# AbrahamSanders/realtime-codec-agent

Hardware: NVIDIA B200
Metric: encode audio-sec/sec (higher is better)
Workload: dtype bf16

## Files before the change

### realtime-codec-agent_b200/csrc/elementwise.cuh

```cuda
#pragma once
#include "gemm_sm100.cuh"

namespace mc {

template <int KT>
__global__ void __launch_bounds__(256)
conv_first_kernel(const float* __restrict__ wav, long long ld, int T, int B, int T0, int s0, int C0,
                  const float* __restrict__ w , const float* __restrict__ bias,
                  __nv_bfloat16* __restrict__ out, int pad_rows) {
  pdl_launch_dependents();
  pdl_wait();
  const int cgroups = C0 / 8;
  const int cg = threadIdx.x % cgroups;
  const int slot = threadIdx.x / cgroups;
  const int frames_per_block = blockDim.x / cgroups;
  float wr[KT][8], br[8];
#pragma unroll
  for (int j = 0; j < KT; ++j) {
    const float4 a = __ldg(reinterpret_cast<const float4*>(w + j * C0 + cg * 8));
    const float4 c = __ldg(reinterpret_cast<const float4*>(w + j * C0 + cg * 8 + 4));
    wr[j][0] = a.x; wr[j][1] = a.y; wr[j][2] = a.z; wr[j][3] = a.w;
    wr[j][4] = c.x; wr[j][5] = c.y; wr[j][6] = c.z; wr[j][7] = c.w;
  }
#pragma unroll
  for (int c = 0; c < 8; ++c) br[c] = __ldg(bias + cg * 8 + c);
  const long long total = static_cast<long long>(B) * T0;
  for (long long bt = blockIdx.x * static_cast<long long>(frames_per_block) + slot; bt < total;
       bt += static_cast<long long>(gridDim.x) * frames_per_block) {
    const int t = static_cast<int>(bt % T0);
    const int b = static_cast<int>(bt / T0);
    const float* x = wav + b * ld;
    float acc[8];
#pragma unroll
    for (int c = 0; c < 8; ++c) acc[c] = br[c];
#pragma unroll
    for (int j = 0; j < KT; ++j) {
      const int n = t * s0 + j - s0;
      const float xv = (n >= 0 && n < T) ? __ldg(x + n) : 0.0f;
#pragma unroll
      for (int c = 0; c < 8; ++c) acc[c] = fmaf(xv, wr[j][c], acc[c]);
    }
    uint4 o;
    o.x = pack_bf16x2(gelu_tanh_f(acc[0]), gelu_tanh_f(acc[1]));
    o.y = pack_bf16x2(gelu_tanh_f(acc[2]), gelu_tanh_f(acc[3]));
    o.z = pack_bf16x2(gelu_tanh_f(acc[4]), gelu_tanh_f(acc[5]));
    o.w = pack_bf16x2(gelu_tanh_f(acc[6]), gelu_tanh_f(acc[7]));
    __nv_bfloat16* dst = out + ((static_cast<long long>(b) * (pad_rows + T0) + pad_rows + t) * C0 + cg * 8);
    *reinterpret_cast<uint4*>(dst) = o;
  }
}

__global__ void rmsnorm_kernel(const float* __restrict__ x, const float* __restrict__ gamma,
                               __nv_bfloat16* __restrict__ out, int M, int d, float eps, int grp_in,
                               long long grp_stride, long long grp_off) {
  pdl_launch_dependents();
  pdl_wait();
  const int warps_per_block = blockDim.x >> 5;
  const int lane = threadIdx.x & 31;
  for (int row = blockIdx.x * warps_per_block + (threadIdx.x >> 5); row < M; row += gridDim.x * warps_per_block) {
    const float4* xr = reinterpret_cast<const float4*>(x + static_cast<long long>(row) * d);
    const int n4 = d >> 2;
    float ss = 0.0f;
    for (int i = lane; i < n4; i += 32) {
      const float4 v = xr[i];
      ss += v.x * v.x + v.y * v.y + v.z * v.z + v.w * v.w;
    }
#pragma unroll
    for (int o = 16; o > 0; o >>= 1) ss += __shfl_xor_sync(0xffffffffu, ss, o);
    const float inv = rsqrtf(ss / static_cast<float>(d) + eps);
    const int grp = row / grp_in;
    const long long obase = static_cast<long long>(grp) * grp_stride + grp_off + static_cast<long long>(row - grp * grp_in) * d;
    uint2* orow_p = reinterpret_cast<uint2*>(out + obase);
    const float4* g4 = reinterpret_cast<const float4*>(gamma);
    for (int i = lane; i < n4; i += 32) {
      const float4 v = xr[i];
      const float4 g = __ldg(g4 + i);
      uint2 o;
      o.x = pack_bf16x2(v.x * inv * g.x, v.y * inv * g.y);
      o.y = pack_bf16x2(v.z * inv * g.z, v.w * inv * g.w);
      orow_p[i] = o;
    }
  }
}

template <int NV>
__global__ void __launch_bounds__(256)
rmsnorm_rows_kernel(const float* __restrict__ x, const float* __restrict__ gamma, __nv_bfloat16* __restrict__ out, int M,
                    float eps, int grp_in, long long grp_stride, long long grp_off) {
  pdl_launch_dependents();
  pdl_wait();
  constexpr int d = NV * 128;
  const int warps_per_block = blockDim.x >> 5;
  const int lane = threadIdx.x & 31;
  float4 g[NV];
#pragma unroll
  for (int u = 0; u < NV; ++u) g[u] = __ldg(reinterpret_cast<const float4*>(gamma) + lane + 32 * u);
  for (int row = blockIdx.x * warps_per_block + (threadIdx.x >> 5); row < M; row += gridDim.x * warps_per_block) {
    const float4* xr = reinterpret_cast<const float4*>(x + static_cast<long long>(row) * d);
    float4 v[NV];
#pragma unroll
    for (int u = 0; u < NV; ++u) v[u] = xr[lane + 32 * u];
    float ss = 0.0f;
#pragma unroll
    for (int u = 0; u < NV; ++u) ss += v[u].x * v[u].x + v[u].y * v[u].y + v[u].z * v[u].z + v[u].w * v[u].w;
#pragma unroll
    for (int o = 16; o > 0; o >>= 1) ss += __shfl_xor_sync(0xffffffffu, ss, o);
    const float inv = rsqrtf(ss / static_cast<float>(d) + eps);
    const int grp = row / grp_in;
    const long long obase = static_cast<long long>(grp) * grp_stride + grp_off + static_cast<long long>(row - grp * grp_in) * d;
    uint2* orow_p = reinterpret_cast<uint2*>(out + obase);
#pragma unroll
    for (int u = 0; u < NV; ++u) {
      uint2 o;
      o.x = pack_bf16x2(v[u].x * inv * g[u].x, v[u].y * inv * g[u].y);
      o.y = pack_bf16x2(v[u].z * inv * g[u].z, v[u].w * inv * g[u].w);
      orow_p[lane + 32 * u] = o;
    }
  }
}

__global__ void compact_rows_kernel(const float4* __restrict__ x, float4* __restrict__ y, int B, int r_in, int r_out,
                                    int d4) {
  pdl_launch_dependents();
  pdl_wait();
  const long long total = static_cast<long long>(B) * r_out * d4;
  for (long long idx = blockIdx.x * static_cast<long long>(blockDim.x) + threadIdx.x; idx < total;
       idx += static_cast<long long>(gridDim.x) * blockDim.x) {
    const int c = static_cast<int>(idx % d4);
    const long long row = idx / d4;
    const int j = static_cast<int>(row % r_out);
    const long long b = row / r_out;
    y[idx] = x[(b * r_in + (r_in - r_out) + j) * d4 + c];
  }
}

__global__ void gather_stem_kernel(const float4* __restrict__ stem, float4* __restrict__ x, int B, int F, int pre,
                                   int fstep, int d4) {
  pdl_launch_dependents();
  pdl_wait();
  const int per = F - pre;
  const long long total = static_cast<long long>(B) * per * d4;
  for (long long idx = blockIdx.x * static_cast<long long>(blockDim.x) + threadIdx.x; idx < total;
       idx += static_cast<long long>(gridDim.x) * blockDim.x) {
    const int c = static_cast<int>(idx % d4);
    const long long row = idx / d4;
    const int t = pre + static_cast<int>(row % per);
    const long long b = row / per;
    x[(b * F + t) * d4 + c] = __ldg(stem + (b * fstep + t) * d4 + c);
  }
}

__global__ void embed_codes_kernel(const long long* __restrict__ codes, const float* __restrict__ table ,
                                   int K, __nv_bfloat16* __restrict__ out, long long M) {
  pdl_launch_dependents();
  pdl_wait();
  const long long total = M * 8;
  for (long long idx = blockIdx.x * static_cast<long long>(blockDim.x) + threadIdx.x; idx < total;
       idx += static_cast<long long>(gridDim.x) * blockDim.x) {
    const long long m = idx >> 3;
    const int piece = static_cast<int>(idx & 7);
    uint4 o = make_uint4(0, 0, 0, 0);
    if (piece < 2) {
      long long code = codes[m];
      code = code < 0 ? 0 : (code >= K ? K - 1 : code);
      const float4* src = reinterpret_cast<const float4*>(table + code * 16 + piece * 8);
      const float4 a = __ldg(src), b = __ldg(src + 1);
      o.x = pack_bf16x2(a.x, a.y);
      o.y = pack_bf16x2(a.z, a.w);
      o.z = pack_bf16x2(b.x, b.y);
      o.w = pack_bf16x2(b.z, b.w);
    }
    *reinterpret_cast<uint4*>(out + m * 64 + piece * 8) = o;
  }
}

__global__ void pack_latents_kernel(const float* __restrict__ z , __nv_bfloat16* __restrict__ out,
                                    long long M) {
  const long long total = M * 8;
  for (long long idx = blockIdx.x * static_cast<long long>(blockDim.x) + threadIdx.x; idx < total;
       idx += static_cast<long long>(gridDim.x) * blockDim.x) {
    const long long m = idx >> 3;
    const int piece = static_cast<int>(idx & 7);
    uint4 o = make_uint4(0, 0, 0, 0);
    if (piece < 2) {
      const float4* src = reinterpret_cast<const float4*>(z + m * 16 + piece * 8);
      const float4 a = src[0], b = src[1];
      o.x = pack_bf16x2(a.x, a.y);
      o.y = pack_bf16x2(a.z, a.w);
      o.z = pack_bf16x2(b.x, b.y);
      o.w = pack_bf16x2(b.z, b.w);
    }
    *reinterpret_cast<uint4*>(out + m * 64 + piece * 8) = o;
  }
}

template <int MAXS>
__global__ void tconv_last_kernel(const __nv_bfloat16* __restrict__ x, int B, int Tin, int Cin, int s,
                                  const float* __restrict__ w , const float* __restrict__ bias,
                                  float* __restrict__ out, int keep) {
  pdl_launch_dependents();
  pdl_wait();
  extern __shared__ float sw[];
  for (int i = threadIdx.x; i < Cin * 2 * s; i += blockDim.x) sw[i] = w[i];
  __syncthreads();
  const float bias0 = __ldg(bias);
  const long long total = static_cast<long long>(B) * Tin;
  const int first_kept = Tin * s - keep;
  for (long long idx = blockIdx.x * static_cast<long long>(blockDim.x) + threadIdx.x; idx < total;
       idx += static_cast<long long>(gridDim.x) * blockDim.x) {
    const int t = static_cast<int>(idx % Tin);
    const int b = static_cast<int>(idx / Tin);
    if ((t + 1) * s <= first_kept) continue;
    const __nv_bfloat16* cur = x + (static_cast<long long>(b) * (Tin + 1) + 1 + t) * Cin;
    const __nv_bfloat16* prev = cur - Cin;
    float acc[MAXS];
#pragma unroll
    for (int j = 0; j < MAXS; ++j) acc[j] = bias0;
    for (int c0 = 0; c0 < Cin; c0 += 8) {
      const uint4 cu = *reinterpret_cast<const uint4*>(cur + c0);
      const uint4 pu = *reinterpret_cast<const uint4*>(prev + c0);
      const __nv_bfloat162* c2 = reinterpret_cast<const __nv_bfloat162*>(&cu);
      const __nv_bfloat162* p2 = reinterpret_cast<const __nv_bfloat162*>(&pu);
#pragma unroll
      for (int u = 0; u < 4; ++u) {
        const float2 cf = __bfloat1622float2(c2[u]);
        const float2 pf = __bfloat1622float2(p2[u]);
        const float* w0 = sw + (c0 + 2 * u) * 2 * s;
        const float* w1 = w0 + 2 * s;
#pragma unroll
        for (int j = 0; j < MAXS; ++j) {
          if (j < s) {
            acc[j] = fmaf(cf.x, w0[j], acc[j]);
            acc[j] = fmaf(pf.x, w0[j + s], acc[j]);
            acc[j] = fmaf(cf.y, w1[j], acc[j]);
            acc[j] = fmaf(pf.y, w1[j + s], acc[j]);
          }
        }
      }
    }
    float* o = out + static_cast<long long>(b) * keep;
#pragma unroll
    for (int j = 0; j < MAXS; ++j) {
      const int n = t * s + j - first_kept;
      if (j < s && n >= 0) o[n] = acc[j];
    }
  }
}

struct PadList {
  int n = 0;
  unsigned char* base[8];
  long long pitch[8];
  int width[8];
};

__global__ void __launch_bounds__(256)
zero_pads_kernel(const PadList pl, int items) {
  pdl_launch_dependents();
  pdl_wait();
  for (int b = 0; b < pl.n; ++b) {
    const int chunks = pl.width[b] >> 4;
    const long long total = static_cast<long long>(items) * chunks;
    for (long long i = blockIdx.x * static_cast<long long>(blockDim.x) + threadIdx.x; i < total;
         i += static_cast<long long>(gridDim.x) * blockDim.x) {
      const long long item = i / chunks;
      const int c = static_cast<int>(i - item * chunks);
      *reinterpret_cast<uint4*>(pl.base[b] + item * pl.pitch[b] + (static_cast<long long>(c) << 4)) = make_uint4(0, 0, 0, 0);
    }
  }
}

__global__ void __launch_bounds__(256)
rowstats_cast_kernel(const float* __restrict__ x, const float* __restrict__ gamma, __nv_bfloat16* __restrict__ xb,
                     float* __restrict__ stats, long long M, int d) {
  pdl_launch_dependents();
  pdl_wait();
  const int nst = d >> 6;
  const long long total = M * nst;
  for (long long i = blockIdx.x * static_cast<long long>(blockDim.x) + threadIdx.x; i < total;
       i += static_cast<long long>(gridDim.x) * blockDim.x) {
    const long long row = i / nst;
    const int c = static_cast<int>(i - row * nst);
    const float4* src = reinterpret_cast<const float4*>(x + row * d + c * 64);
    const float4* gsrc = reinterpret_cast<const float4*>(gamma + c * 64);
    float v[64];
#pragma unroll
    for (int j = 0; j < 16; ++j) {
      const float4 a = src[j];
      v[4 * j] = a.x; v[4 * j + 1] = a.y; v[4 * j + 2] = a.z; v[4 * j + 3] = a.w;
    }
    float ss = 0.f;
#pragma unroll
    for (int j = 0; j < 64; ++j) ss = fmaf(v[j], v[j], ss);
    uint4* dst = reinterpret_cast<uint4*>(xb + row * d + c * 64);
#pragma unroll
    for (int j = 0; j < 8; ++j) {
      const float4 g0 = __ldg(gsrc + 2 * j), g1 = __ldg(gsrc + 2 * j + 1);
      uint4 w;
      w.x = pack_bf16x2(__fmul_rn(v[8 * j], g0.x), __fmul_rn(v[8 * j + 1], g0.y));
      w.y = pack_bf16x2(__fmul_rn(v[8 * j + 2], g0.z), __fmul_rn(v[8 * j + 3], g0.w));
      w.z = pack_bf16x2(__fmul_rn(v[8 * j + 4], g1.x), __fmul_rn(v[8 * j + 5], g1.y));
      w.w = pack_bf16x2(__fmul_rn(v[8 * j + 6], g1.z), __fmul_rn(v[8 * j + 7], g1.w));
      dst[j] = w;
    }
    stats[i] = ss;
  }
}

}
```

### realtime-codec-agent_b200/csrc/engine.cu

```cuda
#include "engine_common.cuh"

#include "attn_sm100.cuh"
#include "attn_vq_simt.cuh"
#include "elementwise.cuh"
#include "gemm_sm100.cuh"
#include "gemm_splitk_sm100.cuh"
#include "ingest.cuh"
#include "post_sm100.cuh"
#include "vq_sm100.cuh"

using namespace mc;
using namespace mc_internal;

namespace {

struct GemmCall {
  const bf16* A; int64_t a_rows; int a_k_wrap;
  const bf16* W; const float* bias;
  int M, N, K, act, out_mode;
  void* out; int64_t ldo;
  int grp_in = INT_MAX, grp_valid = INT_MAX; int64_t grp_stride = 0, grp_off = 0;
  int rope_cols = 0, rope_period = 0, rope_offset = 0;
  int block_n = 0;
  const void* prefetch_ptr = nullptr;
  long long prefetch_bytes = 0;
  const float* row_stats = nullptr; int row_stats_n = 0;
  bf16* xb_out = nullptr; const float* xb_gamma = nullptr; float* stat_out = nullptr;
};

void fill_norm_fields(const mc_handle* h, const GemmCall& c, GemmParams& p) {
  p.row_stats = c.row_stats; p.row_stats_n = c.row_stats_n;
  p.norm_eps = h->spec.norm_eps; p.inv_norm_dim = c.K > 0 ? 1.0f / (float)c.K : 0.f;
  p.xb_out = c.xb_out; p.xb_gamma = c.xb_gamma; p.stat_out = c.stat_out;
}

template <int BN, int BM = GEMM_BM, int KPS = 1>
int launch_gemm_bn(mc_handle* h, const GemmCall& c, cudaStream_t stream) {
  const CUtensorMap *ma, *mb;
  MC_TRY(get_map_2d_bf16(h, c.A, (uint64_t)c.a_k_wrap, (uint64_t)c.a_rows, GEMM_BK, BM, &ma));
  MC_TRY(get_map_2d_bf16(h, c.W, (uint64_t)c.K, (uint64_t)c.N, GEMM_BK, BN, &mb));
  const bool tma_out = (c.grp_in == INT_MAX) && BM == GEMM_BM && c.xb_out == nullptr;
  const CUtensorMap* mo = ma;
  if (tma_out) {
    const int esize = c.out_mode == OUT_BF16 ? 2 : 4;
    MC_TRY(get_map_2d(h, c.out, esize, (uint64_t)c.N, (uint64_t)c.M, (uint64_t)c.ldo * esize, esize == 2 ? 64 : 32, 32, &mo));
  }
  GemmParams p;
  p.tma_store = tma_out ? 1 : 0;
  p.M = c.M; p.N = c.N; p.K = c.K; p.a_k_wrap = c.a_k_wrap;
  p.bias = c.bias; p.act = c.act; p.out_mode = c.out_mode; p.out = c.out; p.ldo = c.ldo;
  p.grp_in = c.grp_in; p.grp_valid = c.grp_valid; p.grp_stride = c.grp_stride; p.grp_off = c.grp_off;
  p.rope_cols = c.rope_cols; p.rope_period = c.rope_period; p.rope_offset = c.rope_offset;
  p.rope_ld = h->spec.max_positions;
  p.rope_cos = c.rope_period > 0 ? h->ptr<float>("rope.cos") : nullptr;
  p.rope_sin = c.rope_period > 0 ? h->ptr<float>("rope.sin") : nullptr;
  fill_norm_fields(h, c, p);
  MC_TRY(mc_allow_smem(h, (gemm_bf16_sm100_kernel<BN, BM, KPS>), GemmCfg<BN>::kSmemBytes));
  const int m_tiles = (c.M + BM - 1) / BM, n_tiles = (c.N + BN - 1) / BN;
  const int grid = std::min(m_tiles * n_tiles, h->num_sms);
  const double valid_rows = c.grp_in == INT_MAX ? (double)c.M : (double)c.M / c.grp_in * c.grp_valid;
  const double out_bytes = valid_rows * c.N * (c.out_mode == OUT_BF16 ? 2.0 : (c.out_mode == OUT_F32 ? 4.0 : 8.0));
  McProfScope prof(h, 0, 2.0 * valid_rows * c.N * c.K, valid_rows * c.a_k_wrap * 2.0 + (double)c.N * c.K * 2.0 + out_bytes, stream);
  mc_launch(h, gemm_bf16_sm100_kernel<BN, BM, KPS>, dim3(grid), dim3(GEMM_THREADS), GemmCfg<BN>::kSmemBytes, stream, *ma, *mb, *mo, p);
  MC_LAUNCH_CHECK(h, "gemm_bf16_sm100_kernel");
  return MC_OK;
}

template <int EPI>
int launch_gemm_pair_epi(mc_handle* h, const GemmParams& p, const CUtensorMap* ma, const CUtensorMap* mb,
                         const CUtensorMap* mo, const CUtensorMap* mo2, int pairs, cudaStream_t stream) {
  constexpr int BN = 256;
  MC_TRY(mc_allow_smem(h, gemm2_bf16_sm100_kernel<BN, EPI>, Gemm2Cfg<BN, EPI>::kSmemBytes));
  mc_launch(h, gemm2_bf16_sm100_kernel<BN, EPI>, dim3(2 * pairs), dim3(GEMM_THREADS), Gemm2Cfg<BN, EPI>::kSmemBytes, stream, *ma, *mb,
            *mo, *mo2, p);
  MC_LAUNCH_CHECK(h, "gemm2_bf16_sm100_kernel");
  return MC_OK;
}

int launch_gemm_pair(mc_handle* h, const GemmCall& c, cudaStream_t stream) {
  constexpr int BN = 256;
  const CUtensorMap *ma, *mb;
  MC_TRY(get_map_2d_bf16(h, c.A, (uint64_t)c.a_k_wrap, (uint64_t)c.a_rows, GEMM_BK, GEMM_BM, &ma));
  MC_TRY(get_map_2d_bf16(h, c.W, (uint64_t)c.K, (uint64_t)c.N, GEMM_BK, BN / 2, &mb));
  const bool norm_fast = c.xb_out != nullptr && h->fast_epilogue && c.grp_in == INT_MAX && c.bias != nullptr && c.N % BN == 0 &&
                         c.out_mode == OUT_F32_RESIDUAL && c.act == ACT_NONE && c.rope_period == 0 && c.ldo == c.N;
  const bool tma_out = (c.grp_in == INT_MAX) && (c.xb_out == nullptr || norm_fast);
  const CUtensorMap* mo = ma;
  const CUtensorMap* mo2 = ma;
  if (tma_out) {
    const int esize = c.out_mode == OUT_BF16 ? 2 : 4;
    MC_TRY(get_map_2d(h, c.out, esize, (uint64_t)c.N, (uint64_t)c.M, (uint64_t)c.ldo * esize, esize == 2 ? 64 : 32, 32, &mo));
  }
  if (norm_fast) MC_TRY(get_map_2d(h, c.xb_out, 2, (uint64_t)c.N, (uint64_t)c.M, (uint64_t)c.N * 2, 64, 32, &mo2));
  GemmParams p;
  p.tma_store = tma_out ? 1 : 0;
  p.M = c.M; p.N = c.N; p.K = c.K; p.a_k_wrap = c.a_k_wrap;
  p.bias = c.bias; p.act = c.act; p.out_mode = c.out_mode; p.out = c.out; p.ldo = c.ldo;
  p.grp_in = c.grp_in; p.grp_valid = c.grp_valid; p.grp_stride = c.grp_stride; p.grp_off = c.grp_off;
  p.rope_cols = c.rope_cols; p.rope_period = c.rope_period; p.rope_offset = c.rope_offset;
  p.rope_ld = h->spec.max_positions;
  p.rope_cos = c.rope_period > 0 ? h->ptr<float>("rope.cos") : nullptr;
  p.rope_sin = c.rope_period > 0 ? h->ptr<float>("rope.sin") : nullptr;
  fill_norm_fields(h, c, p);
  const int m_tiles = (c.M + 2 * GEMM_BM - 1) / (2 * GEMM_BM), n_tiles = (c.N + BN - 1) / BN;
  const int pairs = std::min(m_tiles * n_tiles, h->num_sms / 2);
  const double valid_rows = c.grp_in == INT_MAX ? (double)c.M : (double)c.M / c.grp_in * c.grp_valid;
  const double out_bytes = valid_rows * c.N * (c.out_mode == OUT_BF16 ? 2.0 : (c.out_mode == OUT_F32 ? 4.0 : 8.0));
  McProfScope prof(h, 0, 2.0 * valid_rows * c.N * c.K, valid_rows * c.a_k_wrap * 2.0 + (double)c.N * c.K * 2.0 + out_bytes, stream);
  const bool fast_ok = h->fast_epilogue && tma_out && c.bias != nullptr && c.N % BN == 0;
  if (norm_fast) return launch_gemm_pair_epi<EPI_RESID_NORM>(h, p, ma, mb, mo, mo2, pairs, stream);
  if (fast_ok && c.out_mode == OUT_BF16 && c.act == ACT_NONE && c.rope_period > 0 && c.rope_cols % 64 == 0)
    return launch_gemm_pair_epi<EPI_ROPE_BF16>(h, p, ma, mb, mo, mo2, pairs, stream);
  if (fast_ok && c.out_mode == OUT_BF16 && c.act == ACT_GELU_TANH && c.rope_period == 0)
    return launch_gemm_pair_epi<EPI_GELU_BF16>(h, p, ma, mb, mo, mo2, pairs, stream);
  if (fast_ok && c.out_mode == OUT_F32_RESIDUAL && c.act == ACT_NONE && c.rope_period == 0 && c.xb_out == nullptr)
    return launch_gemm_pair_epi<EPI_RESID_F32>(h, p, ma, mb, mo, mo2, pairs, stream);
  return launch_gemm_pair_epi<EPI_GENERIC>(h, p, ma, mb, mo, mo2, pairs, stream);
}

template <int S>
int launch_gemm_splitk_s(mc_handle* h, const GemmCall& c, cudaStream_t stream) {
  constexpr int BN = 64;
  const CUtensorMap *ma, *mb;
  MC_TRY(get_map_2d_bf16(h, c.A, (uint64_t)c.a_k_wrap, (uint64_t)c.a_rows, GEMM_BK, GEMM_BM, &ma));
  MC_TRY(get_map_2d_bf16(h, c.W, (uint64_t)c.K, (uint64_t)c.N, GEMM_BK, BN, &mb));
  GemmParams p;
  p.tma_store = 0;
  p.M = c.M; p.N = c.N; p.K = c.K; p.a_k_wrap = c.a_k_wrap;
  p.bias = c.bias; p.act = c.act; p.out_mode = c.out_mode; p.out = c.out; p.ldo = c.ldo;
  p.grp_in = c.grp_in; p.grp_valid = c.grp_valid; p.grp_stride = c.grp_stride; p.grp_off = c.grp_off;
  p.rope_cols = c.rope_cols; p.rope_period = c.rope_period; p.rope_offset = c.rope_offset;
  p.rope_ld = h->spec.max_positions;
  p.rope_cos = c.rope_period > 0 ? h->ptr<float>("rope.cos") : nullptr;
  p.rope_sin = c.rope_period > 0 ? h->ptr<float>("rope.sin") : nullptr;
  if (h->l2_prefetch) { p.prefetch_ptr = c.prefetch_ptr; p.prefetch_bytes = c.prefetch_bytes; }
  fill_norm_fields(h, c, p);
  auto kernel = gemm_splitk_sm100_kernel<BN, S>;
  MC_TRY(mc_allow_smem(h, kernel, GemmSkCfg<BN>::kSmemBytes));
  const int m_tiles = (c.M + GEMM_BM - 1) / GEMM_BM, n_tiles = (c.N + BN - 1) / BN;
  const double valid_rows = c.grp_in == INT_MAX ? (double)c.M : (double)c.M / c.grp_in * c.grp_valid;
  const double out_bytes = valid_rows * c.N * (c.out_mode == OUT_BF16 ? 2.0 : (c.out_mode == OUT_F32 ? 4.0 : 8.0));
  McProfScope prof(h, 0, 2.0 * valid_rows * c.N * c.K, valid_rows * c.a_k_wrap * 2.0 + (double)c.N * c.K * 2.0 + out_bytes, stream);
  cudaLaunchConfig_t cfg = {};
  cfg.gridDim = dim3(m_tiles * n_tiles * S); cfg.blockDim = dim3(GEMM_THREADS);
  cfg.dynamicSmemBytes = GemmSkCfg<BN>::kSmemBytes; cfg.stream = stream;
  cudaLaunchAttribute at[2];
  at[0].id = cudaLaunchAttributeClusterDimension;
  at[0].val.clusterDim.x = S; at[0].val.clusterDim.y = 1; at[0].val.clusterDim.z = 1;
  at[1].id = cudaLaunchAttributeProgrammaticStreamSerialization;
  at[1].val.programmaticStreamSerializationAllowed = 1;
  cfg.attrs = at;
  cfg.numAttrs = h->pdl ? 2 : 1;
  const int nkb = (c.K / GEMM_BK) / S;
  const int kps = 1;
  (void)nkb;
  (void)cudaLaunchKernelEx(&cfg, kernel, *ma, *mb, p, kps);
  MC_LAUNCH_CHECK(h, "gemm_splitk_sm100_kernel");
  return MC_OK;
}

int pick_split_k(const mc_handle* h, const GemmCall& c) {
  if (c.M > 2 * GEMM_BM) return 0;
  const int base = ((c.M + GEMM_BM - 1) / GEMM_BM) * ((c.N + 63) / 64);
  const int num_kb = c.K / GEMM_BK;
  if (base > 32) {
    if (base <= 48 && num_kb >= 32 && num_kb % 4 == 0) return 4;
    return 0;
  }
  for (int s = 8; s >= 2; s >>= 1)
    if (num_kb % s == 0 && num_kb / s >= 2 && base * s <= h->num_sms) return s;
  return 0;
}

int launch_gemm_splitk(mc_handle* h, const GemmCall& c, int S, cudaStream_t stream) {
  if (c.rope_period > 0 && c.rope_cols % 64 != 0) return h->fail(MC_ERR_ARG, "split-K gemm: rope needs 64-wide heads");
  if ((c.K / GEMM_BK) % S != 0) return h->fail(MC_ERR_ARG, "split-K gemm: %d k-blocks do not split %d ways", c.K / GEMM_BK, S);
  switch (S) {
    case 2: return launch_gemm_splitk_s<2>(h, c, stream);
    case 4: return launch_gemm_splitk_s<4>(h, c, stream);
    case 8: return launch_gemm_splitk_s<8>(h, c, stream);
    default: return h->fail(MC_ERR_ARG, "split-K gemm: unsupported split %d", S);
  }
}

int launch_gemm(mc_handle* h, const GemmCall& c, cudaStream_t stream) {
  if (c.K % GEMM_BK != 0 || c.K % c.a_k_wrap != 0 || c.a_k_wrap % GEMM_BK != 0)
    return h->fail(MC_ERR_ARG, "gemm: K=%d a_k_wrap=%d must be multiples of %d", c.K, c.a_k_wrap, GEMM_BK);
  if (c.N % 8 != 0) return h->fail(MC_ERR_ARG, "gemm: N=%d must be a multiple of 8", c.N);
  if (c.rope_period > 0 && c.rope_period + c.rope_offset > h->spec.max_positions)
    return h->fail(MC_ERR_ARG, "gemm: rope period %d exceeds table rows %d", c.rope_period, h->spec.max_positions);
  int bn = c.block_n;
  if (c.xb_out && (c.out_mode == OUT_BF16 || c.N % 64 != 0 || !c.xb_gamma || !c.stat_out))
    return h->fail(MC_ERR_ARG, "gemm: fused RMSNorm producer needs an fp32 output, N %% 64 == 0, gamma and a stats buffer");
  if (bn >= 1002 && bn <= 1008) return launch_gemm_splitk(h, c, bn - 1000, stream);
  if (bn == 4064 && (c.K / GEMM_BK) % 4 == 0) return launch_gemm_bn<64, GEMM_BM, 4>(h, c, stream);
  if (bn == 0 && (h->split_k == 2 || (h->split_k == 1 && h->in_session))) {
    const int S = pick_split_k(h, c);
    if (S >= 2) return launch_gemm_splitk(h, c, S, stream);
  }
  {
    const int m2 = (c.M + 255) / 256, n2 = (c.N + 255) / 256;
    if ((bn == 0 && h->gemm_pair && c.N >= 256 && m2 * n2 >= h->num_sms / 2) || bn == 512) return launch_gemm_pair(h, c, stream);
  }
  if (bn == 0) {
    const int m_tiles = (c.M + GEMM_BM - 1) / GEMM_BM;
    if (c.N >= 256 && m_tiles * ((c.N + 255) / 256) >= 2 * h->num_sms) bn = 256;
    else if (c.N >= 128 && m_tiles * ((c.N + 127) / 128) >= h->num_sms) bn = 128;
    else if (c.N >= 256 && m_tiles * ((c.N + 255) / 256) >= h->num_sms) bn = 256;
    else bn = 64;
  }
  if (bn == 64 && c.block_n == 0 && (c.K / GEMM_BK) % 4 == 0 &&
      ((c.M + GEMM_BM - 1) / GEMM_BM) * ((c.N + 63) / 64) <= h->num_sms)
    return launch_gemm_bn<64, GEMM_BM, 4>(h, c, stream);
  switch (bn) {
    case 256: return launch_gemm_bn<256>(h, c, stream);
    case 128: return launch_gemm_bn<128>(h, c, stream);
    case 64: return launch_gemm_bn<64>(h, c, stream);
    default: return h->fail(MC_ERR_ARG, "gemm: unsupported block_n %d", bn);
  }
}

int ew_grid(mc_handle* h, long long work_items, int threads) {
  long long blocks = (work_items + threads - 1) / threads;
  const long long cap = (long long)h->num_sms * 16;
  if (blocks > cap) blocks = cap;
  if (blocks < 1) blocks = 1;
  return (int)blocks;
}

int launch_rmsnorm(mc_handle* h, const float* x, const float* gamma, bf16* out, int M, int d, int grp_in,
                   int64_t grp_stride, int64_t grp_off, cudaStream_t stream) {
  if (d % 4 != 0) return h->fail(MC_ERR_ARG, "rmsnorm: d=%d must be a multiple of 4", d);
  const int warps = 8;
  const int grid = ew_grid(h, M, warps);
  McProfScope prof(h, 3, 0.0, (double)M * d * 6.0, stream);
  const float eps = h->spec.norm_eps;
  switch (d % 128 == 0 ? d / 128 : 0) {
    case 1: mc_launch(h, rmsnorm_rows_kernel<1>, dim3(grid), dim3(warps * 32), 0, stream, x, gamma, out, M, eps, grp_in, (long long)grp_stride, (long long)grp_off); break;
    case 2: mc_launch(h, rmsnorm_rows_kernel<2>, dim3(grid), dim3(warps * 32), 0, stream, x, gamma, out, M, eps, grp_in, (long long)grp_stride, (long long)grp_off); break;
    case 4: mc_launch(h, rmsnorm_rows_kernel<4>, dim3(grid), dim3(warps * 32), 0, stream, x, gamma, out, M, eps, grp_in, (long long)grp_stride, (long long)grp_off); break;
    case 8: mc_launch(h, rmsnorm_rows_kernel<8>, dim3(grid), dim3(warps * 32), 0, stream, x, gamma, out, M, eps, grp_in, (long long)grp_stride, (long long)grp_off); break;
    default: mc_launch(h, rmsnorm_kernel, dim3(grid), dim3(warps * 32), 0, stream, x, gamma, out, M, d, eps, grp_in, (long long)grp_stride, (long long)grp_off);
  }
  MC_LAUNCH_CHECK(h, "rmsnorm_kernel");
  return MC_OK;
}

int launch_attention(mc_handle* h, const bf16* qkv, bf16* out, int B, int F, int out_rows, int phase, int impl, cudaStream_t stream) {
  if (out_rows < 1 || out_rows > F) return h->fail(MC_ERR_ARG, "attention: out_rows %d not in 1 .. %d", out_rows, F);
  const mc_spec& s = h->spec;
  const double span = std::min(F, s.window_left + s.window_right + 1);
  McProfScope prof(h, 1, 4.0 * B * out_rows * span * s.d_model,
                   (double)B * (F * 2.0 + out_rows * 2.0) * s.d_model * 2.0, stream);
  if (impl == 0 && attn_sm100_supported(s.window_left, s.window_right)) {
    MC_TRY(launch_attention_sm100_v3(h, qkv, out, B, F, out_rows, phase, stream));
    return MC_OK;
  }
  if (impl != 0 && impl != 1) return h->fail(MC_ERR_ARG, "attention: unknown implementation %d (0 = tcgen05, 1 = SIMT cross-check)", impl);
  if (s.window_left + s.window_right + 1 > 160) return h->fail(MC_ERR_ARG, "attention window too wide");
  const long long warps = (long long)B * F * s.n_heads;
  const int threads = 256;
  const long long blocks = (warps * 32 + threads - 1) / threads;
  attention_window_simt_kernel<<<(unsigned)blocks, threads, 0, stream>>>(qkv, out, B, F, s.n_heads, s.window_left,
                                                                         s.window_right, out_rows, 0.125f);
  MC_LAUNCH_CHECK(h, "attention_window_simt_kernel");
  return MC_OK;
}

struct StackBufs {
  float* x;
  float* x2;
  bf16* hbuf;
  bf16* qkv;
  bf16* att;
  bf16* ffn;
  float* stats;
};

bool few_rows_regime(const mc_handle* h, long long M) {
  return (h->split_k == 2 || (h->split_k == 1 && h->in_session)) && M <= 2 * GEMM_BM;
}
bool fuse_norm_ok(const mc_handle* h, long long M) {
  if (h->spec.d_model % 64 != 0 || h->fuse_norm == 0) return false;
  return h->fuse_norm >= 2 || few_rows_regime(h, M);
}

int launch_rowstats(mc_handle* h, const float* x, const float* gamma, bf16* xb, float* stats, long long M, int d, cudaStream_t stream) {
  McProfScope prof(h, 3, 0.0, (double)M * d * 6.0, stream);
  mc_launch(h, rowstats_cast_kernel, dim3(ew_grid(h, M * (d / 64), 256)), dim3(256), 0, stream, x, gamma, xb, stats, M, d);
  MC_LAUNCH_CHECK(h, "rowstats_cast_kernel");
  return MC_OK;
}

int run_layers(mc_handle* h, const char* prefix, int n_layers, const StackBufs& b, int B, int F, int keep_rows,
               float** x_out, cudaStream_t stream, int fuse_mode = 0 ,
               const float* final_gamma = nullptr, bf16** xb_out = nullptr, float** stats_out = nullptr) {
  const mc_spec& s = h->spec;
  const int d = s.d_model, f = s.ffn_dim;
  const int nst = d / 64;
  const bool fused = fuse_mode == 1;
  const bool fused2 = fuse_mode != 0;
  std::vector<int> r_in(n_layers), r_out(n_layers);
  {
    int need = std::max(1, std::min(keep_rows, F));
    if (B == 1 && F <= GEMM_BM) need = F;
    for (int l = n_layers - 1; l >= 0; --l) {
      r_out[l] = need;
      need = (need >= F) ? F : std::min(F, need + s.window_left);
      if (!h->exact_cut && need < F) need = F - ((F - need) / 16) * 16;
      r_in[l] = need;
    }
  }
  float* x = b.x;
  float* xalt = b.x2;
  int rows = F;
  char name[128];
  for (int l = 0; l < n_layers; ++l) {
    auto T = [&](const char* leaf) {
      snprintf(name, sizeof(name), "%s.layers.%d.%s", prefix, l, leaf);
      return std::string(name);
    };
    const int Ri = rows, Ro = std::min(r_out[l], rows);
    const int Mi = B * Ri, Mo = B * Ro;
    if (!fused) MC_TRY(launch_rmsnorm(h, x, h->ptr<float>(T("norm1")), b.hbuf, Mi, d, INT_MAX, 0, 0, stream));
    GemmCall g{};
    if (fused) { g.row_stats = b.stats; g.row_stats_n = nst; }
    g.A = b.hbuf; g.a_rows = Mi; g.a_k_wrap = d; g.W = h->ptr<bf16>(T("wqkv")); g.bias = h->ptr<float>(T("bqkv"));
    g.M = Mi; g.N = 3 * d; g.K = d; g.act = ACT_NONE; g.out_mode = OUT_BF16; g.out = b.qkv; g.ldo = 3 * d;
    g.rope_cols = 2 * d; g.rope_period = Ri; g.rope_offset = F - Ri;
    g.prefetch_ptr = h->ptr<bf16>(T("wo")); g.prefetch_bytes = (long long)d * d * 2;
    MC_TRY(launch_gemm(h, g, stream));
    MC_TRY(launch_attention(h, b.qkv, b.att, B, Ri, Ro, (F - Ri) % 16, h->attn_impl, stream));
    if (Ro < Ri) {
      const long long items = (long long)Mo * (d / 4);
      McProfScope prof(h, 3, 0.0, (double)Mo * d * 8.0, stream);
      mc_launch(h, compact_rows_kernel, dim3(ew_grid(h, items, 256)), dim3(256), 0, stream, reinterpret_cast<const float4*>(x),
                reinterpret_cast<float4*>(xalt), B, Ri, Ro, d / 4);
      MC_LAUNCH_CHECK(h, "compact_rows_kernel");
      std::swap(x, xalt);
      rows = Ro;
    }
    GemmCall o{};
    o.A = b.att; o.a_rows = Mo; o.a_k_wrap = d; o.W = h->ptr<bf16>(T("wo")); o.bias = h->ptr<float>(T("bo"));
    o.M = Mo; o.N = d; o.K = d; o.act = ACT_NONE; o.out_mode = OUT_F32_RESIDUAL; o.out = x; o.ldo = d;
    o.prefetch_ptr = h->ptr<bf16>(T("w1")); o.prefetch_bytes = (long long)f * d * 2;
    if (fused2) { o.xb_out = b.hbuf; o.xb_gamma = h->ptr<float>(T("norm2")); o.stat_out = b.stats; }
    MC_TRY(launch_gemm(h, o, stream));
    if (!fused2) MC_TRY(launch_rmsnorm(h, x, h->ptr<float>(T("norm2")), b.hbuf, Mo, d, INT_MAX, 0, 0, stream));
    GemmCall u{};
    if (fused2) { u.row_stats = b.stats; u.row_stats_n = nst; }
    u.A = b.hbuf; u.a_rows = Mo; u.a_k_wrap = d; u.W = h->ptr<bf16>(T("w1")); u.bias = h->ptr<float>(T("b1"));
    u.M = Mo; u.N = f; u.K = d; u.act = ACT_GELU_TANH; u.out_mode = OUT_BF16; u.out = b.ffn; u.ldo = f;
    u.prefetch_ptr = h->ptr<bf16>(T("w2")); u.prefetch_bytes = (long long)d * f * 2;
    MC_TRY(launch_gemm(h, u, stream));
    GemmCall w{};
    w.A = b.ffn; w.a_rows = Mo; w.a_k_wrap = f; w.W = h->ptr<bf16>(T("w2")); w.bias = h->ptr<float>(T("b2"));
    w.M = Mo; w.N = d; w.K = f; w.act = ACT_NONE; w.out_mode = OUT_F32_RESIDUAL; w.out = x; w.ldo = d;
    if (l + 1 < n_layers) {
      snprintf(name, sizeof(name), "%s.layers.%d.wqkv", prefix, l + 1);
      w.prefetch_ptr = h->ptr<bf16>(name); w.prefetch_bytes = (long long)3 * d * d * 2;
    }
    if (fused) {
      const float* next_gamma = final_gamma;
      if (l + 1 < n_layers) {
        snprintf(name, sizeof(name), "%s.layers.%d.norm1", prefix, l + 1);
        next_gamma = h->ptr<float>(name);
      }
      if (next_gamma) { w.xb_out = b.hbuf; w.xb_gamma = next_gamma; w.stat_out = b.stats; }
    }
    MC_TRY(launch_gemm(h, w, stream));
  }
  bf16* xb = b.hbuf;
  float* st = b.stats;
  if (rows > keep_rows && B == 1) {
    x += (size_t)(rows - keep_rows) * d;
    xb += (size_t)(rows - keep_rows) * d;
    st += (size_t)(rows - keep_rows) * nst;
  } else if (rows > keep_rows) {
    const int Ro = keep_rows;
    const long long items = (long long)B * Ro * (d / 4);
    mc_launch(h, compact_rows_kernel, dim3(ew_grid(h, items, 256)), dim3(256), 0, stream, reinterpret_cast<const float4*>(x),
              reinterpret_cast<float4*>(xalt), B, rows, Ro, d / 4);
    MC_LAUNCH_CHECK(h, "compact_rows_kernel");
    std::swap(x, xalt);
  }
  if (fused && final_gamma && rows > keep_rows && B != 1) return h->fail(MC_ERR_STATE, "run_layers: fused norms with a trailing compaction");
  *x_out = x;
  if (xb_out) *xb_out = xb;
  if (stats_out) *stats_out = st;
  return MC_OK;
}

StackBufs carve_stack(Carver& cv, uint8_t* base, int M, int d, int f, bool dry) {
  StackBufs b{};
  size_t ox = cv.take((size_t)M * d * 4), ox2 = cv.take((size_t)M * d * 4), oh = cv.take((size_t)M * d * 2),
         oq = cv.take((size_t)M * 3 * d * 2), oa = cv.take((size_t)M * d * 2), of = cv.take((size_t)M * f * 2),
         os = cv.take((size_t)M * (d / 64 + 1) * 4);
  if (!dry) {
    b.stats = reinterpret_cast<float*>(base + os);
    b.x = reinterpret_cast<float*>(base + ox);
    b.x2 = reinterpret_cast<float*>(base + ox2);
    b.hbuf = reinterpret_cast<bf16*>(base + oh);
    b.qkv = reinterpret_cast<bf16*>(base + oq);
    b.att = reinterpret_cast<bf16*>(base + oa);
    b.ffn = reinterpret_cast<bf16*>(base + of);
  }
  return b;
}

int launch_vq(mc_handle* h, const float* z, int n_items, int F, int keep, int64_t* codes, float* margin,
              void* scratch, cudaStream_t stream);
size_t vq_scratch_bytes(mc_handle* h, int Mq);

struct ConvPlan {
  int B = 0, T = 0;
  std::vector<int> Tl;
  std::vector<size_t> off;
};

ConvPlan plan_conv(const mc_spec& s, Carver& cv, int Bc, int Tc_padded) {
  ConvPlan p;
  p.B = Bc; p.T = Tc_padded;
  const int n = s.n_convs;
  p.Tl.resize(n); p.off.resize(n);
  int t = Tc_padded;
  for (int i = 0; i < n; ++i) { t /= s.conv_strides[i]; p.Tl[i] = t; }
  for (int i = 0; i + 1 < n; ++i)
    p.off[i] = cv.take((size_t)Bc * (s.conv_strides[i + 1] + p.Tl[i]) * s.conv_channels[i] * 2 + 65536);
  return p;
}

int run_conv_stack(mc_handle* h, const ConvPlan& cp, uint8_t* base, const float* wav, int64_t ld, int Tvalid,
                   float* x_out, int64_t x_item_stride, cudaStream_t stream, bf16* xb_out = nullptr,
                   const float* xb_gamma = nullptr, float* stat_out = nullptr) {
  const mc_spec& s = h->spec;
  const int n = s.n_convs, d = s.d_model, B = cp.B;
  const std::vector<int>& Tl = cp.Tl;
  const int* Cl = s.conv_channels;
  {
    PadList pl;
    long long work = 0;
    for (int i = 0; i + 1 < n; ++i) {
      const int pad = s.conv_strides[i + 1];
      pl.base[pl.n] = base + cp.off[i];
      pl.pitch[pl.n] = (long long)(pad + Tl[i]) * Cl[i] * 2;
      pl.width[pl.n] = pad * Cl[i] * 2;
      if (pl.width[pl.n] % 16 != 0 || pl.pitch[pl.n] % 16 != 0) return h->fail(MC_ERR_ARG, "conv %d: padding is not 16-byte granular", i + 1);
      work = std::max(work, (long long)B * (pl.width[pl.n] >> 4));
      ++pl.n;
    }
    if (pl.n > 0) {
      mc_launch(h, zero_pads_kernel, dim3(ew_grid(h, work, 256)), dim3(256), 0, stream, pl, B);
      MC_LAUNCH_CHECK(h, "zero_pads_kernel");
    }
  }
  {
    const int s0 = s.conv_strides[0], C0 = Cl[0];
    const int cgroups = C0 / 8;
    if ((2 * s0 != 8 && 2 * s0 != 16) || C0 % 8 != 0 || 256 % cgroups != 0)
      return h->fail(MC_ERR_ARG, "conv0: stride %d / channels %d unsupported", s0, C0);
    const int threads = 256;
    const long long frames = (long long)B * Tl[0];
    const int grid = ew_grid(h, frames * cgroups, threads);
    McProfScope prof(h, 3, 2.0 * B * Tl[0] * 2 * s0 * C0, (double)B * Tvalid * 4.0 + (double)B * Tl[0] * C0 * 2.0, stream);
    bf16* o0 = reinterpret_cast<bf16*>(base + cp.off[0]);
    if (2 * s0 == 8)
      mc_launch(h, conv_first_kernel<8>, dim3(grid), dim3(threads), 0, stream, wav, (long long)ld, Tvalid, B, Tl[0], s0, C0,
                h->ptr<float>("enc.conv0.w"), h->ptr<float>("enc.conv0.b"), o0, (int)s.conv_strides[1]);
    else
      mc_launch(h, conv_first_kernel<16>, dim3(grid), dim3(threads), 0, stream, wav, (long long)ld, Tvalid, B, Tl[0], s0, C0,
                h->ptr<float>("enc.conv0.w"), h->ptr<float>("enc.conv0.b"), o0, (int)s.conv_strides[1]);
    MC_LAUNCH_CHECK(h, "conv_first_kernel");
  }
  for (int i = 1; i < n; ++i) {
    const int si = s.conv_strides[i];
    const long long rows = (long long)B * (1 + Tl[i]);
    if (rows > INT_MAX) return h->fail(MC_ERR_ARG, "encode: conv %d has too many rows", i);
    GemmCall g{};
    g.A = reinterpret_cast<const bf16*>(base + cp.off[i - 1]);
    g.a_k_wrap = si * Cl[i - 1];
    g.a_rows = rows;
    g.W = h->ptr<bf16>("enc.conv" + std::to_string(i) + ".w");
    g.bias = h->ptr<float>("enc.conv" + std::to_string(i) + ".b");
    g.M = (int)rows; g.N = Cl[i]; g.K = 2 * g.a_k_wrap;
    g.grp_in = 1 + Tl[i]; g.grp_valid = Tl[i];
    if (i + 1 < n) {
      const int pad = s.conv_strides[i + 1];
      g.act = ACT_GELU_TANH; g.out_mode = OUT_BF16; g.out = base + cp.off[i]; g.ldo = Cl[i];
      g.grp_stride = (int64_t)(pad + Tl[i]) * Cl[i]; g.grp_off = (int64_t)pad * Cl[i];
    } else {
      g.act = ACT_NONE; g.out_mode = OUT_F32; g.out = x_out; g.ldo = d;
      g.grp_stride = x_item_stride; g.grp_off = 0;
      g.xb_out = xb_out; g.xb_gamma = xb_gamma; g.stat_out = stat_out;
    }
    MC_TRY(launch_gemm(h, g, stream));
  }
  return MC_OK;
}

int stem_prefix_frames(const mc_spec& s) {
  long long dirty = 0;
  for (int i = 0; i < s.n_convs; ++i) {
    const int st = s.conv_strides[i];
    dirty = (dirty + st - 1) / st + 1;
  }
  return (int)dirty;
}

struct RaggedKeep {
  const int* rtable;
  int C, keep;
};

int encode_impl(mc_handle* h, const float* wav, int64_t ld, int B, int T, int keep, int64_t* codes, float* margin,
                float* z_e_out, cudaStream_t stream, const RaggedKeep* ragged = nullptr) {
  const mc_spec& s = h->spec;
  const int n = s.n_convs;
  int hop = 1;
  for (int i = 0; i < n; ++i) hop *= s.conv_strides[i];
  const int F = (T + hop - 1) / hop;
  if (F < 1) return h->fail(MC_ERR_ARG, "encode: empty input");
  if (F > s.max_positions) return h->fail(MC_ERR_ARG, "encode: %d frames exceed RoPE table (%d rows)", F, s.max_positions);
  if (keep <= 0 || keep > F) keep = F;
  const int Tp = F * hop;
  const int d = s.d_model, dq = s.codebook_dim;
  const long long Mll = (long long)B * F;
  if (Mll * std::max(3 * d, s.ffn_dim) > (long long)INT_MAX) return h->fail(MC_ERR_ARG, "encode: batch too large");
  const int M = (int)Mll;

  const int pre = stem_prefix_frames(s);
  const long long span_samples = (long long)(B - 1) * ld + T;
  const long long span_frames = span_samples / hop;
  const bool shared = h->shared_stem && B >= 2 && ld > 0 && ld < T && ld % hop == 0 && T % hop == 0 && F > pre &&
                      span_samples <= INT_MAX && span_frames + (long long)pre * B < (long long)B * F / 2;
  const int fuse_mode = !(fuse_norm_ok(h, Mll + B) && s.enc_layers > 0) ? 0 : ((h->fuse_norm == 3 && !few_rows_regime(h, Mll + B)) ? 2 : 1);
  const bool fused = fuse_mode == 1;
  const bool conv_producer = fused && few_rows_regime(h, Mll + B) && !shared;

  Carver cv;
  ConvPlan cp_full, cp_span, cp_pre;
  size_t ostem = 0;
  if (shared) {
    cp_span = plan_conv(s, cv, 1, (int)span_samples);
    cp_pre = plan_conv(s, cv, B, pre * hop);
    ostem = cv.take((size_t)span_frames * d * 4);
  } else {
    cp_full = plan_conv(s, cv, B, Tp);
  }
  Carver cv2 = cv;
  carve_stack(cv2, nullptr, M, d, s.ffn_dim, true);
  size_t oz = cv2.take((size_t)M * dq * 4);
  size_t ovq = cv2.take(vq_scratch_bytes(h, B * keep));
  const size_t ozg = ragged ? cv2.take((size_t)B * ragged->keep * dq * 4) : 0;
  MC_TRY(arena_reserve(h, cv2.off, stream));
  uint8_t* base = h->arena;
  StackBufs sb = carve_stack(cv, base, M, d, s.ffn_dim, false);
  float* z_e = reinterpret_cast<float*>(base + oz);
  void* vq_scratch = base + ovq;

  if (shared) {
    float* stem = reinterpret_cast<float*>(base + ostem);
    MC_TRY(run_conv_stack(h, cp_span, base, wav, span_samples, (int)span_samples, stem, 0, stream));
    MC_TRY(run_conv_stack(h, cp_pre, base, wav, ld, pre * hop, sb.x, (int64_t)F * d, stream));
    const long long items = (long long)B * (F - pre) * (d / 4);
    McProfScope prof(h, 3, 0.0, (double)B * (F - pre) * d * 8.0, stream);
    mc_launch(h, gather_stem_kernel, dim3(ew_grid(h, items, 256)), dim3(256), 0, stream, reinterpret_cast<const float4*>(stem),
              reinterpret_cast<float4*>(sb.x), B, F, pre, (int)(ld / hop), d / 4);
    MC_LAUNCH_CHECK(h, "gather_stem_kernel");
  } else {
    if (conv_producer)
      MC_TRY(run_conv_stack(h, cp_full, base, wav, ld, T, sb.x, (int64_t)F * d, stream, sb.hbuf, h->ptr<float>("enc.layers.0.norm1"), sb.stats));
    else
      MC_TRY(run_conv_stack(h, cp_full, base, wav, ld, T, sb.x, (int64_t)F * d, stream));
  }
  if (fused && !conv_producer) MC_TRY(launch_rowstats(h, sb.x, h->ptr<float>("enc.layers.0.norm1"), sb.hbuf, sb.stats, M, d, stream));
  const int keep_rows = z_e_out ? F : keep;
  float* xk = nullptr;
  bf16* xbk = sb.hbuf;
  float* stk = nullptr;
  MC_TRY(run_layers(h, "enc", s.enc_layers, sb, B, F, keep_rows, &xk, stream, fuse_mode, fused ? h->ptr<float>("enc.norm_f") : nullptr, &xbk, &stk));
  const int Mk = B * keep_rows;
  if (!fused) MC_TRY(launch_rmsnorm(h, xk, h->ptr<float>("enc.norm_f"), sb.hbuf, Mk, d, INT_MAX, 0, 0, stream));
  GemmCall pj{};
  if (fused) { pj.row_stats = stk; pj.row_stats_n = d / 64; }
  pj.A = fused ? xbk : sb.hbuf; pj.a_rows = Mk; pj.a_k_wrap = d; pj.W = h->ptr<bf16>("enc.proj.w"); pj.bias = h->ptr<float>("enc.proj.b");
  pj.M = Mk; pj.N = dq; pj.K = d; pj.act = ACT_NONE; pj.out_mode = OUT_F32; pj.out = z_e; pj.ldo = dq;
  MC_TRY(launch_gemm(h, pj, stream));
  if (z_e_out) MC_CUDA(h, cudaMemcpyAsync(z_e_out, z_e, (size_t)M * dq * 4, cudaMemcpyDeviceToDevice, stream));
  if (ragged) {
    float* zg = reinterpret_cast<float*>(base + ozg);
    pool_gather_rows_ragged_kernel<<<dim3(1, B), 256, 0, stream>>>(z_e, ragged->rtable, ragged->C, keep_rows, F, ragged->keep,
                                                                   dq, hop, zg);
    MC_LAUNCH_CHECK(h, "pool_gather_rows_ragged_kernel");
    return launch_vq(h, zg, B, ragged->keep, ragged->keep, codes, margin, vq_scratch, stream);
  }
  MC_TRY(launch_vq(h, z_e, B, keep_rows, keep, codes, margin, vq_scratch, stream));
  return MC_OK;
}

int decode_impl(mc_handle* h, const int64_t* codes, const float* z_q, int B, int F, int keep, float* wav,
                cudaStream_t stream) {
  const mc_spec& s = h->spec;
  const int n = s.n_convs;
  if (F < 1 || B < 1) return h->fail(MC_ERR_ARG, "decode: empty input");
  if (F > s.max_positions) return h->fail(MC_ERR_ARG, "decode: %d frames exceed RoPE table (%d rows)", F, s.max_positions);
  int hop = 1;
  for (int i = 0; i < n; ++i) hop *= s.conv_strides[i];
  const int d = s.d_model;
  const long long Mll = (long long)B * F;
  if (Mll * std::max(3 * d, s.ffn_dim) > (long long)INT_MAX) return h->fail(MC_ERR_ARG, "decode: batch too large");
  const int M = (int)Mll;
  const int total = F * hop;
  if (keep <= 0 || keep > total) keep = total;
  std::vector<int> dch(n + 1), ds(n), Tin(n);
  dch[0] = d;
  for (int i = 0; i < n; ++i) {
    ds[i] = s.conv_strides[n - 1 - i];
    dch[i + 1] = (n - 2 - i >= 0) ? s.conv_channels[n - 2 - i] : 1;
  }
  const int Rk = (keep >= total) ? F : std::min(F, (keep + hop - 1) / hop + 2);
  Tin[0] = Rk;
  for (int i = 1; i < n; ++i) Tin[i] = Tin[i - 1] * ds[i - 1];

  Carver cv;
  size_t oa0 = cv.take((size_t)M * 64 * 2);
  std::vector<size_t> tb_off(n);
  for (int i = 0; i < n; ++i) tb_off[i] = cv.take((size_t)B * (1 + Tin[i]) * dch[i] * 2 + 65536);
  Carver cv2 = cv;
  carve_stack(cv2, nullptr, M, d, s.ffn_dim, true);
  MC_TRY(arena_reserve(h, cv2.off, stream));
  uint8_t* base = h->arena;
  StackBufs sb = carve_stack(cv, base, M, d, s.ffn_dim, false);
  bf16* a0 = reinterpret_cast<bf16*>(base + oa0);

  const int threads = 256;
  if (codes) {
    mc_launch(h, embed_codes_kernel, dim3(ew_grid(h, (long long)M * 8, threads)), dim3(threads), 0, stream,
              reinterpret_cast<const long long*>(codes), h->ptr<float>("vq.codebook"), (int)s.codebook_size, a0, (long long)M);
    MC_LAUNCH_CHECK(h, "embed_codes_kernel");
  } else {
    pack_latents_kernel<<<ew_grid(h, (long long)M * 8, threads), threads, 0, stream>>>(z_q, a0, M);
    MC_LAUNCH_CHECK(h, "pack_latents_kernel");
  }
  GemmCall ip{};
  ip.A = a0; ip.a_rows = M; ip.a_k_wrap = 64; ip.W = h->ptr<bf16>("dec.in_proj.w"); ip.bias = h->ptr<float>("dec.in_proj.b");
  ip.M = M; ip.N = d; ip.K = 64; ip.act = ACT_NONE; ip.out_mode = OUT_F32; ip.out = sb.x; ip.ldo = d;
  const int fuse_mode = !(fuse_norm_ok(h, Mll) && s.dec_layers > 0) ? 0 : ((h->fuse_norm == 3 && !few_rows_regime(h, Mll)) ? 2 : 1);
  const bool fused = fuse_mode == 1;
  const bool proj_producer = fused && few_rows_regime(h, Mll);
  if (proj_producer) { ip.xb_out = sb.hbuf; ip.xb_gamma = h->ptr<float>("dec.layers.0.norm1"); ip.stat_out = sb.stats; }
  MC_TRY(launch_gemm(h, ip, stream));
  if (fused && !proj_producer) MC_TRY(launch_rowstats(h, sb.x, h->ptr<float>("dec.layers.0.norm1"), sb.hbuf, sb.stats, M, d, stream));
  float* xk = nullptr;
  MC_TRY(run_layers(h, "dec", s.dec_layers, sb, B, F, Rk, &xk, stream, fuse_mode));

  {
    PadList pl;
    long long work = 0;
    for (int i = 0; i < n; ++i) {
      pl.base[pl.n] = base + tb_off[i];
      pl.pitch[pl.n] = (long long)(1 + Tin[i]) * dch[i] * 2;
      pl.width[pl.n] = dch[i] * 2;
      if (pl.width[pl.n] % 16 != 0) return h->fail(MC_ERR_ARG, "tconv %d: %d channels are not 16-byte granular", i, dch[i]);
      work = std::max(work, (long long)B * (pl.width[pl.n] >> 4));
      ++pl.n;
    }
    mc_launch(h, zero_pads_kernel, dim3(ew_grid(h, work, 256)), dim3(256), 0, stream, pl, B);
    MC_LAUNCH_CHECK(h, "zero_pads_kernel");
  }
  MC_TRY(launch_rmsnorm(h, xk, h->ptr<float>("dec.norm_f"), reinterpret_cast<bf16*>(base + tb_off[0]), B * Rk, d, Rk,
                        (int64_t)(1 + Rk) * d, d, stream));
  for (int i = 0; i + 1 < n; ++i) {
    GemmCall g{};
    g.A = reinterpret_cast<const bf16*>(base + tb_off[i]);
    g.a_k_wrap = dch[i]; g.a_rows = (int64_t)B * (1 + Tin[i]);
    g.W = h->ptr<bf16>("dec.up" + std::to_string(i) + ".w");
    g.bias = h->ptr<float>("dec.up" + std::to_string(i) + ".b");
    g.M = B * (1 + Tin[i]); g.N = ds[i] * dch[i + 1]; g.K = 2 * dch[i];
    g.grp_in = 1 + Tin[i]; g.grp_valid = Tin[i];
    g.act = ACT_GELU_TANH; g.out_mode = OUT_BF16; g.out = base + tb_off[i + 1]; g.ldo = g.N;
    g.grp_stride = (int64_t)(1 + Tin[i + 1]) * dch[i + 1]; g.grp_off = dch[i + 1];
    MC_TRY(launch_gemm(h, g, stream));
  }
  {
    const int i = n - 1;
    if (ds[i] > 8 || dch[i] % 8 != 0) return h->fail(MC_ERR_ARG, "last tconv: stride %d / channels %d unsupported", ds[i], dch[i]);
    const long long items = (long long)B * Tin[i];
    const size_t smem = (size_t)dch[i] * 2 * ds[i] * 4;
    McProfScope prof(h, 3, 4.0 * B * Tin[i] * dch[i] * ds[i], (double)B * Tin[i] * dch[i] * 2.0 + (double)B * keep * 4.0, stream);
    mc_launch(h, tconv_last_kernel<8>, dim3(ew_grid(h, items, threads)), dim3(threads), smem, stream,
              reinterpret_cast<const bf16*>(base + tb_off[i]), B, Tin[i], dch[i], ds[i],
              h->ptr<float>("dec.up" + std::to_string(i) + ".w"), h->ptr<float>("dec.up" + std::to_string(i) + ".b"), wav, keep);
    MC_LAUNCH_CHECK(h, "tconv_last_kernel");
  }
  return MC_OK;
}

size_t vq_scratch_bytes(mc_handle* h, int Mq) {
  return std::max(vq_sm100_scratch_bytes(h->num_sms, Mq), (size_t)64 * Mq * sizeof(VqPartial)) + 1024;
}

int launch_vq(mc_handle* h, const float* z, int n_items, int F, int keep, int64_t* codes, float* margin,
              void* scratch, cudaStream_t stream) {
  const mc_spec& s = h->spec;
  const int Mq = n_items * keep;
  McProfScope prof(h, 2, 2.0 * Mq * (double)s.codebook_size * s.codebook_dim, (double)s.codebook_size * 128.0, stream);
  if (h->vq_impl == 0) {
    return launch_vq_sm100(h, z, n_items, F, keep, codes, margin, scratch, stream);
  }
  const int row_tiles = (Mq + 127) / 128;
  int splits = (2 * h->num_sms + row_tiles - 1) / row_tiles;
  splits = std::max(1, std::min(64, splits));
  vq_simt_kernel<<<dim3(row_tiles, splits), 128, 0, stream>>>(z, Mq, F, keep, h->ptr<float>("vq.codebook"),
                                                              h->ptr<float>("vq.c2"), s.codebook_size, splits,
                                                              reinterpret_cast<VqPartial*>(scratch));
  MC_LAUNCH_CHECK(h, "vq_simt_kernel");
  vq_merge_kernel<<<(Mq + 255) / 256, 256, 0, stream>>>(reinterpret_cast<const VqPartial*>(scratch), Mq, splits,
                                                        reinterpret_cast<long long*>(codes), margin);
  MC_LAUNCH_CHECK(h, "vq_merge_kernel");
  return MC_OK;
}

std::vector<std::string> required_tensors(const mc_spec& s) {
  std::vector<std::string> v;
  const int n = s.n_convs;
  for (int i = 0; i < n; ++i) {
    v.push_back("enc.conv" + std::to_string(i) + ".w");
    v.push_back("enc.conv" + std::to_string(i) + ".b");
    v.push_back("dec.up" + std::to_string(i) + ".w");
    v.push_back("dec.up" + std::to_string(i) + ".b");
  }
  const char* leaves[] = {"norm1", "wqkv", "bqkv", "wo", "bo", "norm2", "w1", "b1", "w2", "b2"};
  for (int st = 0; st < 2; ++st)
    for (int l = 0; l < (st == 0 ? s.enc_layers : s.dec_layers); ++l)
      for (const char* leaf : leaves)
        v.push_back(std::string(st == 0 ? "enc" : "dec") + ".layers." + std::to_string(l) + "." + leaf);
  for (const char* nm : {"enc.norm_f", "enc.proj.w", "enc.proj.b", "vq.codebook", "vq.c2", "vq.packed", "dec.in_proj.w",
                         "dec.in_proj.b", "dec.norm_f", "rope.cos", "rope.sin"})
    v.push_back(nm);
  return v;
}

}

extern "C" {

int mc_version(void) { return MC_VERSION; }

const char* mc_last_error(const mc_handle* h) { return h ? h->err.c_str() : g_create_error.c_str(); }

int mc_create(const mc_spec* spec, int device, mc_handle** out) {
  if (!spec || !out) { g_create_error = "mc_create: null argument"; return MC_ERR_ARG; }
  *out = nullptr;
  cudaDeviceProp prop;
  cudaError_t e = cudaGetDeviceProperties(&prop, device);
  if (e != cudaSuccess) { g_create_error = std::string("mc_create: ") + cudaGetErrorString(e); return MC_ERR_CUDA; }
  if (prop.major != 10) {
    g_create_error = "mc_create: device is sm_" + std::to_string(prop.major * 10 + prop.minor) +
                     "; this library contains sm_100a code only (no fallback)";
    return MC_ERR_ARCH;
  }
  if (spec->n_convs < 2 || spec->n_convs > MC_MAX_CONVS || spec->d_model % 64 != 0 || spec->d_model / spec->n_heads != 64 ||
      spec->ffn_dim % 64 != 0 || spec->codebook_dim != 16 || spec->codebook_size % 256 != 0 ||
      spec->conv_channels[spec->n_convs - 1] != spec->d_model) {
    g_create_error = "mc_create: unsupported spec (need head_dim 64, d/ffn multiples of 64, codebook_dim 16)";
    return MC_ERR_ARG;
  }
  e = cudaSetDevice(device);
  if (e != cudaSuccess) { g_create_error = std::string("mc_create: ") + cudaGetErrorString(e); return MC_ERR_CUDA; }
  mc_handle* h = new mc_handle();
  h->spec = *spec;
  h->device = device;
  h->num_sms = prop.multiProcessorCount;
  *out = h;
  return MC_OK;
}

int mc_destroy(mc_handle* h) {
  if (!h) return MC_OK;
  if (h->arena) cudaFree(h->arena);
  delete h;
  return MC_OK;
}

int mc_set_tensor(mc_handle* h, const char* name, const void* dev_ptr, int64_t numel) {
  if (!h || !name || !dev_ptr) return MC_ERR_ARG;
  Tensor t; t.p = dev_ptr; t.numel = numel;
  h->tensors[name] = t;
  h->tensor_gen++;
  h->finalized = false;
  return MC_OK;
}

int mc_finalize(mc_handle* h) {
  if (!h) return MC_ERR_ARG;
  for (const std::string& nm : required_tensors(h->spec))
    if (!h->find(nm)) return h->fail(MC_ERR_ARG, "mc_finalize: tensor '%s' was not registered", nm.c_str());
  h->finalized = true;
  return MC_OK;
}

#define MC_ENTER(h)                                                        \
  if (!(h)) return MC_ERR_ARG;                                             \
  if (!(h)->finalized) return (h)->fail(MC_ERR_STATE, "handle not finalized"); \
  { cudaError_t e__ = cudaSetDevice((h)->device); if (e__ != cudaSuccess) return (h)->fail(MC_ERR_CUDA, "cudaSetDevice failed"); }

int mc_encode(mc_handle* h, const float* wav, int64_t ld, int32_t B, int32_t T, int32_t keep_last_frames,
              int64_t* codes, float* margin, float* z_e, mc_stream_t stream) {
  MC_ENTER(h);
  if (!wav || !codes || B < 1 || T < 1) return h->fail(MC_ERR_ARG, "mc_encode: bad arguments (B=%d T=%d)", B, T);
  return encode_impl(h, wav, ld, B, T, keep_last_frames, codes, margin, z_e, (cudaStream_t)stream);
}

int mc_decode(mc_handle* h, const int64_t* codes, int32_t B, int32_t F, int32_t keep_last_samples, float* wav,
              mc_stream_t stream) {
  MC_ENTER(h);
  if (!codes || !wav) return h->fail(MC_ERR_ARG, "mc_decode: null pointer");
  return decode_impl(h, codes, nullptr, B, F, keep_last_samples, wav, (cudaStream_t)stream);
}

int mc_decode_latents(mc_handle* h, const float* z_q, int32_t B, int32_t F, int32_t keep_last_samples, float* wav,
                      mc_stream_t stream) {
  MC_ENTER(h);
  if (!z_q || !wav) return h->fail(MC_ERR_ARG, "mc_decode_latents: null pointer");
  return decode_impl(h, nullptr, z_q, B, F, keep_last_samples, wav, (cudaStream_t)stream);
}

int mc_vq_search(mc_handle* h, const float* z, int32_t M, int64_t* codes, float* margin, mc_stream_t stream) {
  MC_ENTER(h);
  if (!z || !codes || M < 1) return h->fail(MC_ERR_ARG, "mc_vq_search: bad arguments");
  Carver cv;
  cv.take(vq_scratch_bytes(h, M));
  MC_TRY(arena_reserve(h, cv.off, (cudaStream_t)stream));
  return launch_vq(h, z, M, 1, 1, codes, margin, h->arena, (cudaStream_t)stream);
}

int mc_codebook(mc_handle* h, float* out, mc_stream_t stream) {
  MC_ENTER(h);
  const Tensor* t = h->find("vq.codebook");
  MC_CUDA(h, cudaMemcpyAsync(out, t->p, (size_t)t->numel * 4, cudaMemcpyDeviceToDevice, (cudaStream_t)stream));
  return MC_OK;
}

int mc_embed_distance(mc_handle* h, const int64_t* ids, int32_t rows, int32_t n, int64_t vocab_start, const float* ref,
                      float* dist_out, float* mean_out, mc_stream_t stream) {
  MC_ENTER(h);
  if (!ids || rows < 1 || n < 1 || (!dist_out && !mean_out)) return h->fail(MC_ERR_ARG, "mc_embed_distance: bad arguments");
  embed_distance_kernel<<<rows, POST_THREADS, 0, (cudaStream_t)stream>>>(
      reinterpret_cast<const long long*>(ids), n, (long long)vocab_start, h->ptr<float>("vq.codebook"), h->spec.codebook_size,
      ref, dist_out, mean_out);
  MC_LAUNCH_CHECK(h, "embed_distance_kernel");
  return MC_OK;
}

int mc_op_embed_distance(mc_handle* h, const float* table, int32_t K, const int64_t* ids, int32_t rows, int32_t n,
                         int64_t vocab_start, const float* ref, float* dist_out, float* mean_out, mc_stream_t stream) {
  MC_ENTER(h);
  if (!table || K < 1 || !ids || rows < 1 || n < 1 || (!dist_out && !mean_out))
    return h->fail(MC_ERR_ARG, "mc_op_embed_distance: bad arguments");
  embed_distance_kernel<<<rows, POST_THREADS, 0, (cudaStream_t)stream>>>(reinterpret_cast<const long long*>(ids), n,
                                                                         (long long)vocab_start, table, K, ref, dist_out, mean_out);
  MC_LAUNCH_CHECK(h, "embed_distance_kernel");
  return MC_OK;
}

int mc_op_emit_chunk(mc_handle* h, const float* wav, int32_t n_have, int32_t chunk, int32_t fade, int32_t has_prev,
                     float target_rms, float silence_rms_threshold, const float* fade_in, float* prev_tail, float* out,
                     mc_stream_t stream) {
  MC_ENTER(h);
  if (!wav || !fade_in || !prev_tail || !out || chunk < 1 || fade < 1 || fade > chunk || n_have < 1)
    return h->fail(MC_ERR_ARG, "mc_op_emit_chunk: bad arguments");
  emit_chunk_kernel<<<1, POST_THREADS, 0, (cudaStream_t)stream>>>(wav, n_have, chunk, fade, has_prev, target_rms,
                                                                  silence_rms_threshold, fade_in, prev_tail, out);
  MC_LAUNCH_CHECK(h, "emit_chunk_kernel");
  return MC_OK;
}

int mc_render_chunks(mc_handle* h, const float* windows, int64_t ld, int32_t n_chunks, int32_t chunk, int32_t fade,
                     int32_t last_len, float target_rms, float silence_rms_threshold, const float* fade_in, float* out,
                     mc_stream_t stream) {
  MC_ENTER(h);
  if (!windows || !fade_in || !out || n_chunks < 1 || chunk < 1 || fade < 1 || fade > chunk || last_len < 1 || last_len > chunk ||
      ld < (int64_t)chunk + fade)
    return h->fail(MC_ERR_ARG, "mc_render_chunks: need 0 < fade (%d) <= chunk (%d), 0 < last_len (%d) <= chunk, ld (%lld) >= chunk + fade",
                   fade, chunk, last_len, (long long)ld);
  const double out_n = (double)(n_chunks - 1) * chunk + last_len;
  McProfScope prof(h, 3, 0.0, out_n * 4.0 * 2.0 + (double)n_chunks * fade * 4.0, (cudaStream_t)stream);
  mc_launch(h, emit_chunks_kernel, dim3(n_chunks), dim3(POST_THREADS), 0, (cudaStream_t)stream, windows, (long long)ld, (int)n_chunks,
            (int)chunk, (int)fade, (int)last_len, target_rms, silence_rms_threshold, fade_in, out);
  MC_LAUNCH_CHECK(h, "emit_chunks_kernel");
  return MC_OK;
}

int mc_op_f32_to_pcm(mc_handle* h, const float* in, int64_t in_ld, int32_t channels, int64_t frames, int32_t format, void* out,
                     mc_stream_t stream) {
  MC_ENTER(h);
  if (!in || !out || channels < 1 || frames < 1 || in_ld < frames || (format != PCM_S16 && format != PCM_F32))
    return h->fail(MC_ERR_ARG, "mc_op_f32_to_pcm: bad arguments (format %d, channels %d, frames %lld)", format, channels, (long long)frames);
  if (reinterpret_cast<uintptr_t>(out) & (format == PCM_S16 ? 1 : 3))
    return h->fail(MC_ERR_ARG, "mc_op_f32_to_pcm: output is not naturally aligned");
  McProfScope prof(h, 3, 0.0, (double)frames * channels * (4.0 + (format == PCM_S16 ? 2.0 : 4.0)), (cudaStream_t)stream);
  f32_to_pcm_kernel<<<ew_grid(h, frames * channels, 256), 256, 0, (cudaStream_t)stream>>>(in, (long long)in_ld, channels,
                                                                                          (long long)frames, format, out);
  MC_LAUNCH_CHECK(h, "f32_to_pcm_kernel");
  return MC_OK;
}

int mc_op_pcm_to_f32(mc_handle* h, const void* pcm, int32_t format, int32_t big_endian, int32_t channels, int64_t frames,
                     int32_t mix_mono, float* out, int64_t out_ld, mc_stream_t stream) {
  MC_ENTER(h);
  if (!pcm || !out || channels < 1 || frames < 1 || format < PCM_U8 || format > PCM_ALAW || (!mix_mono && out_ld < frames))
    return h->fail(MC_ERR_ARG, "mc_op_pcm_to_f32: bad arguments (format %d, channels %d, frames %lld)", format, channels, (long long)frames);
  if ((format == PCM_F32 && (reinterpret_cast<uintptr_t>(pcm) & 3)) || (format == PCM_F64 && (reinterpret_cast<uintptr_t>(pcm) & 7)))
    return h->fail(MC_ERR_ARG, "mc_op_pcm_to_f32: float payload is not naturally aligned");
  McProfScope prof(h, 3, 0.0, (double)frames * channels * 2.0 + (double)frames * (mix_mono ? 1 : channels) * 4.0, (cudaStream_t)stream);
  pcm_to_f32_kernel<<<ew_grid(h, frames, 256), 256, 0, (cudaStream_t)stream>>>(
      reinterpret_cast<const unsigned char*>(pcm), format, big_endian, channels, (long long)frames, mix_mono, out, (long long)out_ld);
  MC_LAUNCH_CHECK(h, "pcm_to_f32_kernel");
  return MC_OK;
}

int mc_op_resample(mc_handle* h, const float* in, int64_t in_ld, int32_t channels, int64_t n_in, int32_t up, int32_t down,
                   const float* taps, int32_t n_taps, int64_t pre_remove, float* out, int64_t out_ld, int64_t n_out,
                   mc_stream_t stream) {
  MC_ENTER(h);
  if (!in || !taps || !out || channels < 1 || n_in < 1 || n_out < 1 || up < 1 || down < 1 || n_taps < 1 || pre_remove < 0 ||
      in_ld < n_in || out_ld < n_out)
    return h->fail(MC_ERR_ARG, "mc_op_resample: bad arguments (up %d, down %d, taps %d)", up, down, n_taps);
  McProfScope prof(h, 3, 2.0 * channels * (double)n_out * ((double)n_taps / up), (double)channels * (n_in + n_out) * 4.0, (cudaStream_t)stream);
  resample_poly_kernel<<<ew_grid(h, (long long)channels * n_out, 256), 256, 0, (cudaStream_t)stream>>>(
      in, (long long)in_ld, channels, (long long)n_in, up, down, taps, n_taps, (long long)pre_remove, out, (long long)out_ld,
      (long long)n_out);
  MC_LAUNCH_CHECK(h, "resample_poly_kernel");
  return MC_OK;
}

int64_t mc_debug_trace(mc_handle* h, void* dev_buf, int64_t capacity_records) {
  if (!h) return MC_ERR_ARG;
#ifdef MC_TRACE
  unsigned int n = 0, zero = 0, cap = (unsigned int)capacity_records;
  cudaDeviceSynchronize();
  cudaMemcpyFromSymbol(&n, g_mc_trace_n, sizeof(n));
  unsigned long long* ptr = reinterpret_cast<unsigned long long*>(dev_buf);
  cudaMemcpyToSymbol(g_mc_trace, &ptr, sizeof(ptr));
  cudaMemcpyToSymbol(g_mc_trace_cap, &cap, sizeof(cap));
  cudaMemcpyToSymbol(g_mc_trace_n, &zero, sizeof(zero));
  return (int64_t)n;
#else
  (void)dev_buf; (void)capacity_records;
  return h->fail(MC_ERR_STATE, "mc_debug_trace: the library was built without -DMC_TRACE");
#endif
}

int64_t mc_launch_count(const mc_handle* h) { return h ? h->launches : 0; }

int mc_profile_begin(mc_handle* h) {
  if (!h) return MC_ERR_ARG;
  for (auto& r : h->prof) { h->event_pool.push_back(r.a); h->event_pool.push_back(r.b); }
  h->prof.clear();
  h->profiling = true;
  return MC_OK;
}

int mc_profile_end(mc_handle* h, double* ms, double* flops, double* bytes, int64_t* launches, int32_t n_classes) {
  if (!h || !ms || !flops || !bytes || !launches) return MC_ERR_ARG;
  h->profiling = false;
  for (int c = 0; c < n_classes; ++c) { ms[c] = 0; flops[c] = 0; bytes[c] = 0; launches[c] = 0; }
  for (auto& r : h->prof) {
    cudaError_t e = cudaEventSynchronize(r.b);
    if (e != cudaSuccess) return h->fail(MC_ERR_CUDA, "mc_profile_end: %s", cudaGetErrorString(e));
    float t = 0.f;
    cudaEventElapsedTime(&t, r.a, r.b);
    if (r.cls < n_classes) { ms[r.cls] += t; flops[r.cls] += r.flops; bytes[r.cls] += r.bytes; launches[r.cls]++; }
    h->event_pool.push_back(r.a); h->event_pool.push_back(r.b);
  }
  h->prof.clear();
  return MC_OK;
}

int mc_set_option(mc_handle* h, const char* key, int32_t value) {
  if (!h || !key) return MC_ERR_ARG;
  const std::string k(key);
  if (k == "shared_stem") h->shared_stem = value != 0;
  else if (k == "exact_cut") { h->exact_cut = value != 0; h->tensor_gen++; }
  else if (k == "gemm_pair") h->gemm_pair = value != 0;
  else if (k == "fast_epilogue") h->fast_epilogue = value != 0;
  else if (k == "pdl") h->pdl = value != 0;
  else if (k == "attn_p_tmem") h->attn_p_tmem = value != 0;
  else if (k == "debug_repeat") h->debug_repeat = value;
  else if (k == "l2_prefetch") { h->l2_prefetch = value != 0; h->tensor_gen++; }
  else if (k == "fuse_norm") {
    if (value < 0 || value > 3) return h->fail(MC_ERR_ARG, "mc_set_option: fuse_norm is 0 .. 3");
    h->fuse_norm = value; h->tensor_gen++;
  }
  else if (k == "small_m_split_k") {
    if (value < 0 || value > 2) return h->fail(MC_ERR_ARG, "mc_set_option: small_m_split_k is 0, 1 or 2");
    h->split_k = value;
    h->tensor_gen++;
  }
  else if (k == "max_positions") {
    if (value < 1) return h->fail(MC_ERR_ARG, "mc_set_option: max_positions must be positive");
    h->spec.max_positions = value;
  }
  else return h->fail(MC_ERR_ARG, "mc_set_option: unknown option '%s'", key);
  return MC_OK;
}

int mc_set_debug_impl(mc_handle* h, int32_t attention_impl, int32_t vq_impl) {
  if (!h) return MC_ERR_ARG;
  h->gemm_pair = (attention_impl & 4) ? 0 : 1;
  attention_impl &= 1;
  h->attn_impl = attention_impl;
  h->vq_impl = vq_impl;
  return MC_OK;
}

int mc_op_gemm(mc_handle* h, const void* A, int64_t a_rows, int32_t a_k_wrap, const void* W, const float* bias,
               int32_t M, int32_t N, int32_t K, int32_t act, int32_t out_mode, void* out, int64_t ldo,
               int32_t grp_in, int32_t grp_valid, int64_t grp_stride, int64_t grp_off, int32_t rope_cols,
               int32_t rope_period, int32_t block_n, mc_stream_t stream) {
  MC_ENTER(h);
  GemmCall g{};
  g.A = reinterpret_cast<const bf16*>(A); g.a_rows = a_rows; g.a_k_wrap = a_k_wrap;
  g.W = reinterpret_cast<const bf16*>(W); g.bias = bias; g.M = M; g.N = N; g.K = K; g.act = act; g.out_mode = out_mode;
  g.out = out; g.ldo = ldo;
  g.grp_in = grp_in > 0 ? grp_in : INT_MAX; g.grp_valid = grp_in > 0 ? grp_valid : INT_MAX;
  g.grp_stride = grp_stride; g.grp_off = grp_off;
  g.rope_cols = rope_cols; g.rope_period = rope_period; g.block_n = block_n;
  for (int r = 1; r < h->debug_repeat; ++r) MC_TRY(launch_gemm(h, g, (cudaStream_t)stream));
  return launch_gemm(h, g, (cudaStream_t)stream);
}

int mc_op_gemm_fused(mc_handle* h, const void* A, const void* W, const float* bias, int32_t M, int32_t N, int32_t K, int32_t act,
                     int32_t out_mode, void* out, const float* row_stats, int32_t row_stats_n, void* xb_out, const float* xb_gamma,
                     float* stat_out, int32_t rope_cols, int32_t rope_period, int32_t block_n, mc_stream_t stream) {
  MC_ENTER(h);
  GemmCall g{};
  g.A = reinterpret_cast<const bf16*>(A); g.a_rows = M; g.a_k_wrap = K;
  g.W = reinterpret_cast<const bf16*>(W); g.bias = bias; g.M = M; g.N = N; g.K = K; g.act = act; g.out_mode = out_mode;
  g.out = out; g.ldo = N;
  g.rope_cols = rope_cols; g.rope_period = rope_period; g.block_n = block_n;
  g.row_stats = row_stats; g.row_stats_n = row_stats_n;
  g.xb_out = reinterpret_cast<bf16*>(xb_out); g.xb_gamma = xb_gamma; g.stat_out = stat_out;
  for (int r = 1; r < h->debug_repeat; ++r) MC_TRY(launch_gemm(h, g, (cudaStream_t)stream));
  return launch_gemm(h, g, (cudaStream_t)stream);
}

int mc_op_rowstats(mc_handle* h, const float* x, const float* gamma, void* xb_out, float* stat_out, int32_t M, int32_t d,
                   mc_stream_t stream) {
  MC_ENTER(h);
  if (!x || !gamma || !xb_out || !stat_out || M < 1 || d % 64 != 0) return h->fail(MC_ERR_ARG, "mc_op_rowstats: bad arguments");
  for (int r = 1; r < h->debug_repeat; ++r) MC_TRY(launch_rowstats(h, x, gamma, reinterpret_cast<bf16*>(xb_out), stat_out, M, d, (cudaStream_t)stream));
  return launch_rowstats(h, x, gamma, reinterpret_cast<bf16*>(xb_out), stat_out, M, d, (cudaStream_t)stream);
}

int mc_op_rmsnorm(mc_handle* h, const float* x, const float* gamma, void* out_bf16, int32_t M, int32_t d,
                  mc_stream_t stream) {
  MC_ENTER(h);
  for (int r = 1; r < h->debug_repeat; ++r) MC_TRY(launch_rmsnorm(h, x, gamma, reinterpret_cast<bf16*>(out_bf16), M, d, INT_MAX, 0, 0, (cudaStream_t)stream));
  return launch_rmsnorm(h, x, gamma, reinterpret_cast<bf16*>(out_bf16), M, d, INT_MAX, 0, 0, (cudaStream_t)stream);
}

int mc_op_attention(mc_handle* h, const void* qkv, void* out, int32_t B, int32_t F, int32_t out_rows, int32_t phase,
                    int32_t impl, mc_stream_t stream) {
  MC_ENTER(h);
  for (int r = 1; r < h->debug_repeat; ++r)
    MC_TRY(launch_attention(h, reinterpret_cast<const bf16*>(qkv), reinterpret_cast<bf16*>(out), B, F, out_rows, phase, impl,
                            (cudaStream_t)stream));
  return launch_attention(h, reinterpret_cast<const bf16*>(qkv), reinterpret_cast<bf16*>(out), B, F, out_rows, phase, impl,
                          (cudaStream_t)stream);
}

}

struct mc_stream {
  mc_handle* h = nullptr;
  int C = 1;
  int ctx_samples = 32000, ctx_frames = 100;
  int cap_samples = 0, cap_frames = 0;
  float* audio[2] = {nullptr, nullptr};
  int64_t* codes_ctx[2] = {nullptr, nullptr};
  int audio_len = 0, code_len = 0, acur = 0, ccur = 0;
  int32_t* pin_table = nullptr;
  float* pin_audio = nullptr;
  int64_t* pin_codes = nullptr;
  float* pin_wav = nullptr;
  int64_t* dev_codes_out = nullptr;
  float* dev_wav_out = nullptr;
  struct GraphEntry { cudaGraphExec_t exec = nullptr; int uses = 0; size_t arena_gen = 0; };
  std::map<std::tuple<int, int, int, int, int>, GraphEntry> graphs;
  bool use_graphs = true;
  cudaStream_t own = nullptr;
  cudaEvent_t order_ev = nullptr;
  std::string err;
  int emit_chunk = 0, emit_fade = 0, emit_has_prev = 0;
  float emit_target_rms = 0.f, emit_silence_thr = 0.f;
  float* emit_fade_in = nullptr;
  float* emit_prev_tail = nullptr;
  float* emit_out = nullptr;
  float* pin_emit = nullptr;
};

namespace {

size_t handle_generation(const mc_handle* h) {
  return reinterpret_cast<size_t>(h->arena) ^ h->arena_cap ^ (static_cast<size_t>(h->tensor_gen) << 48);
}

void stream_drop_graphs(mc_stream* s) {
  for (auto& kv : s->graphs)
    if (kv.second.exec) cudaGraphExecDestroy(kv.second.exec);
  s->graphs.clear();
}

template <typename Sess, typename Key, typename Body>
int run_or_replay_impl(Sess* s, Key key, cudaStream_t stream, Body body);

template <typename Sess, typename Key, typename Body>
int run_or_replay(Sess* s, Key key, cudaStream_t stream, Body body) {
  s->h->in_session = true;
  const int rc = run_or_replay_impl(s, key, stream, body);
  s->h->in_session = false;
  return rc;
}

template <typename Sess, typename Key, typename Body>
int run_or_replay_impl(Sess* s, Key key, cudaStream_t stream, Body body) {
  mc_handle* h = s->h;
  if (!s->use_graphs || h->profiling) return body();
  auto& e = s->graphs[key];
  const size_t gen = handle_generation(h);
  if (e.exec && e.arena_gen != gen) {
    cudaGraphExecDestroy(e.exec);
    e.exec = nullptr;
    e.uses = 0;
  }
  if (e.exec) {
    MC_CUDA(h, cudaGraphLaunch(e.exec, stream));
    h->launches += 1;
    return MC_OK;
  }
  if (e.uses++ == 0) return body();
  MC_CUDA(h, cudaStreamBeginCapture(stream, cudaStreamCaptureModeRelaxed));
  const int64_t launches_before = h->launches;
  const int rc = body();
  cudaGraph_t graph = nullptr;
  cudaError_t ce = cudaStreamEndCapture(stream, &graph);
  h->launches = launches_before;
  if (rc != MC_OK || ce != cudaSuccess || graph == nullptr) {
    if (graph) cudaGraphDestroy(graph);
    (void)cudaGetLastError();
    s->use_graphs = false;
    return body();
  }
  ce = cudaGraphInstantiate(&e.exec, graph, 0);
  cudaGraphDestroy(graph);
  if (ce != cudaSuccess) {
    e.exec = nullptr;
    s->use_graphs = false;
    return body();
  }
  e.arena_gen = handle_generation(h);
  MC_CUDA(h, cudaGraphLaunch(e.exec, stream));
  h->launches += 1;
  return MC_OK;
}

}

extern "C" {

int mc_stream_create(mc_handle* h, int32_t channels, int32_t context_samples, int32_t max_chunk_samples, mc_stream** out) {
  MC_ENTER(h);
  if (!out || channels < 1 || context_samples < 1) return h->fail(MC_ERR_ARG, "mc_stream_create: bad arguments");
  int hop = 1;
  for (int i = 0; i < h->spec.n_convs; ++i) hop *= h->spec.conv_strides[i];
  mc_stream* s = new mc_stream();
  s->h = h; s->C = channels;
  s->ctx_samples = context_samples;
  s->ctx_frames = context_samples / hop;
  s->cap_samples = std::max(context_samples, max_chunk_samples);
  s->cap_frames = (s->cap_samples + hop - 1) / hop;
  if (s->cap_frames > h->spec.max_positions) { delete s; return h->fail(MC_ERR_ARG, "mc_stream_create: context exceeds RoPE table"); }
  const size_t ab = (size_t)channels * s->cap_samples * 4, cb = (size_t)channels * s->cap_frames * 8;
  cudaError_t e = cudaSuccess;
  for (int i = 0; i < 2 && e == cudaSuccess; ++i) {
    e = cudaMalloc(&s->audio[i], ab);
    if (e == cudaSuccess) e = cudaMalloc(&s->codes_ctx[i], cb);
  }
  if (e == cudaSuccess) e = cudaMalloc(&s->dev_codes_out, cb);
  if (e == cudaSuccess) e = cudaMalloc(&s->dev_wav_out, ab);
  if (e == cudaSuccess) e = cudaMallocHost(&s->pin_table, 16);
  if (e == cudaSuccess) e = cudaMallocHost(&s->pin_audio, ab);
  if (e == cudaSuccess) e = cudaMallocHost(&s->pin_codes, cb);
  if (e == cudaSuccess) e = cudaMallocHost(&s->pin_wav, ab);
  if (e == cudaSuccess) e = cudaStreamCreateWithFlags(&s->own, cudaStreamNonBlocking);
  if (e == cudaSuccess) e = cudaEventCreateWithFlags(&s->order_ev, cudaEventDisableTiming);
  if (e != cudaSuccess) { mc_stream_destroy(s); return h->fail(MC_ERR_NOMEM, "mc_stream_create: %s", cudaGetErrorString(e)); }
  *out = s;
  return MC_OK;
}

int mc_stream_destroy(mc_stream* s) {
  if (!s) return MC_OK;
  stream_drop_graphs(s);
  for (int i = 0; i < 2; ++i) { if (s->audio[i]) cudaFree(s->audio[i]); if (s->codes_ctx[i]) cudaFree(s->codes_ctx[i]); }
  if (s->dev_codes_out) cudaFree(s->dev_codes_out);
  if (s->dev_wav_out) cudaFree(s->dev_wav_out);
  if (s->pin_table) cudaFreeHost(s->pin_table);
  if (s->pin_audio) cudaFreeHost(s->pin_audio);
  if (s->pin_codes) cudaFreeHost(s->pin_codes);
  if (s->pin_wav) cudaFreeHost(s->pin_wav);
  if (s->emit_fade_in) cudaFree(s->emit_fade_in);
  if (s->emit_prev_tail) cudaFree(s->emit_prev_tail);
  if (s->emit_out) cudaFree(s->emit_out);
  if (s->pin_emit) cudaFreeHost(s->pin_emit);
  if (s->order_ev) cudaEventDestroy(s->order_ev);
  if (s->own) cudaStreamDestroy(s->own);
  delete s;
  return MC_OK;
}

int mc_stream_reset(mc_stream* s) {
  if (!s) return MC_ERR_ARG;
  s->audio_len = 0; s->code_len = 0;
  s->emit_has_prev = 0;
  return MC_OK;
}

int mc_stream_reset_part(mc_stream* s, int32_t audio, int32_t codes) {
  if (!s) return MC_ERR_ARG;
  if (audio) s->audio_len = 0;
  if (codes) s->code_len = 0;
  return MC_OK;
}

int mc_stream_load_audio(mc_stream* s, const float* audio, int32_t n) {
  if (!s) return MC_ERR_ARG;
  mc_handle* h = s->h;
  MC_ENTER(h);
  if (n < 0 || (n > 0 && !audio)) return h->fail(MC_ERR_ARG, "mc_stream_load_audio: bad arguments");
  const int keep = std::min(n, s->ctx_samples);
  MC_CUDA(h, cudaStreamSynchronize(s->own));
  if (keep > 0)
    MC_CUDA(h, cudaMemcpy2D(s->audio[s->acur], (size_t)s->cap_samples * 4, audio + (n - keep), (size_t)n * 4, (size_t)keep * 4,
                            s->C, cudaMemcpyHostToDevice));
  s->audio_len = keep;
  return MC_OK;
}

int mc_stream_load_codes(mc_stream* s, const int64_t* codes, int32_t n) {
  if (!s) return MC_ERR_ARG;
  mc_handle* h = s->h;
  MC_ENTER(h);
  if (n < 0 || (n > 0 && !codes)) return h->fail(MC_ERR_ARG, "mc_stream_load_codes: bad arguments");
  const int keep = std::min(n, s->ctx_frames);
  MC_CUDA(h, cudaStreamSynchronize(s->own));
  if (keep > 0)
    MC_CUDA(h, cudaMemcpy2D(s->codes_ctx[s->ccur], (size_t)s->cap_frames * 8, codes + (n - keep), (size_t)n * 8, (size_t)keep * 8,
                            s->C, cudaMemcpyHostToDevice));
  s->code_len = keep;
  return MC_OK;
}

int mc_stream_push_audio(mc_stream* s, const float* chunk, int32_t n, int32_t keep_frames, int64_t* codes_out,
                         int32_t* frames_out, mc_stream_t stream_) {
  if (!s) return MC_ERR_ARG;
  mc_handle* h = s->h;
  MC_ENTER(h);
  cudaStream_t caller = (cudaStream_t)stream_;
  MC_CUDA(h, cudaEventRecord(s->order_ev, caller));
  MC_CUDA(h, cudaStreamWaitEvent(s->own, s->order_ev, 0));
  cudaStream_t stream = s->own;
  if (!chunk || !codes_out || n < 1) return h->fail(MC_ERR_ARG, "mc_stream_push_audio: bad arguments");
  if (n > s->cap_samples) return h->fail(MC_ERR_ARG, "mc_stream_push_audio: chunk of %d samples exceeds the session capacity %d", n, s->cap_samples);
  int hop = 1;
  for (int i = 0; i < h->spec.n_convs; ++i) hop *= h->spec.conv_strides[i];
  const int C = s->C, cap = s->cap_samples;
  const int new_len = std::min(s->audio_len + n, std::max(n, s->ctx_samples));
  const int keep_old = new_len - n;
  const int F = (new_len + hop - 1) / hop;
  const int keep = (keep_frames <= 0 || keep_frames > F) ? F : keep_frames;
  for (int c = 0; c < C; ++c) memcpy(s->pin_audio + (size_t)c * cap, chunk + (size_t)c * n, (size_t)n * 4);
  const int src = s->acur, dst = s->acur ^ 1;
  const int old_len = s->audio_len;
  s->pin_table[0] = 0; s->pin_table[1] = src;
  auto body = [&]() -> int {
// ... 639 lines not shown
```

### realtime-codec-agent_b200/csrc/engine_common.cuh

```cuda
#pragma once
#include <cuda.h>
#include <cuda_runtime.h>
#include <stdarg.h>
#include <stdio.h>
#include <string.h>

#include <algorithm>
#include <climits>
#include <map>
#include <set>
#include <string>
#include <tuple>
#include <unordered_map>
#include <utility>
#include <vector>

#include "../../include/magicodec_b200.h"
#include "ptx_sm100.cuh"

typedef __nv_bfloat16 bf16;

namespace mc_internal {

inline thread_local std::string g_create_error;

typedef CUresult (*EncodeTiledFn)(CUtensorMap*, CUtensorMapDataType, cuuint32_t, void*, const cuuint64_t*,
                                  const cuuint64_t*, const cuuint32_t*, const cuuint32_t*, CUtensorMapInterleave,
                                  CUtensorMapSwizzle, CUtensorMapL2promotion, CUtensorMapFloatOOBfill);

inline EncodeTiledFn get_encode_fn() {
  static EncodeTiledFn fn = nullptr;
  if (fn == nullptr) {
    void* p = nullptr;
    cudaDriverEntryPointQueryResult q;
    if (cudaGetDriverEntryPoint("cuTensorMapEncodeTiled", &p, cudaEnableDefault, &q) == cudaSuccess &&
        q == cudaDriverEntryPointSuccess) {
      fn = reinterpret_cast<EncodeTiledFn>(p);
    }
  }
  return fn;
}

struct Tensor {
  const void* p = nullptr;
  int64_t numel = 0;
};

}
using mc_internal::Tensor;

struct mc_handle {
  mc_spec spec{};
  int device = 0;
  int num_sms = 148;
  bool finalized = false;
  std::unordered_map<std::string, Tensor> tensors;
  std::string err;
  int64_t launches = 0;
  uint32_t tensor_gen = 0;
  int attn_impl = 0, vq_impl = 0;
  int gemm_pair = 1;
  bool fast_epilogue = true;
  bool attn_p_tmem = true;
  int split_k = 1;
  bool in_session = false;
  int debug_repeat = 1;
  int fuse_norm = 1;
  bool l2_prefetch = true;
  bool pdl = true;
  bool shared_stem = true;
  bool exact_cut = true;
  struct ProfRec { cudaEvent_t a, b; int cls; double flops; double bytes; };
  bool profiling = false;
  std::vector<ProfRec> prof;
  std::vector<cudaEvent_t> event_pool;
  std::set<const void*> smem_configured;
  uint8_t* arena = nullptr;
  size_t arena_cap = 0;
  size_t arena_off = 0;
  std::map<std::tuple<const void*, uint64_t, uint64_t, uint64_t, uint32_t, uint32_t>, CUtensorMap> maps;

  int fail(int code, const char* fmt, ...) {
    char buf[1024];
    va_list ap;
    va_start(ap, fmt);
    vsnprintf(buf, sizeof(buf), fmt, ap);
    va_end(ap);
    err = buf;
    return code;
  }
  const Tensor* find(const std::string& name) const {
    auto it = tensors.find(name);
    return it == tensors.end() ? nullptr : &it->second;
  }
  template <typename T>
  const T* ptr(const std::string& name) const {
    return reinterpret_cast<const T*>(tensors.at(name).p);
  }
};

#define MC_CUDA(h, expr)                                                                         \
  do {                                                                                           \
    cudaError_t e__ = (expr);                                                                    \
    if (e__ != cudaSuccess)                                                                      \
      return (h)->fail(MC_ERR_CUDA, "%s failed: %s (%s:%d)", #expr, cudaGetErrorString(e__), __FILE__, __LINE__); \
  } while (0)
#define MC_TRY(expr)          \
  do {                        \
    int rc__ = (expr);        \
    if (rc__ != MC_OK) return rc__; \
  } while (0)
struct McProfScope {
  mc_handle* h; cudaStream_t st; bool on;
  mc_handle::ProfRec rec;
  static cudaEvent_t get_event(mc_handle* h) {
    if (!h->event_pool.empty()) { cudaEvent_t e = h->event_pool.back(); h->event_pool.pop_back(); return e; }
    cudaEvent_t e; cudaEventCreate(&e); return e;
  }
  McProfScope(mc_handle* h_, int cls, double flops, double bytes, cudaStream_t s) : h(h_), st(s), on(h_->profiling) {
    if (!on) return;
    rec.a = get_event(h); rec.b = get_event(h); rec.cls = cls; rec.flops = flops; rec.bytes = bytes;
    cudaEventRecord(rec.a, st);
  }
  ~McProfScope() {
    if (!on) return;
    cudaEventRecord(rec.b, st);
    h->prof.push_back(rec);
  }
};

template <typename K>
inline int mc_allow_smem(mc_handle* h, K kernel, int bytes) {
  const void* key = reinterpret_cast<const void*>(kernel);
  if (h->smem_configured.count(key)) return MC_OK;
  MC_CUDA(h, cudaFuncSetAttribute(kernel, cudaFuncAttributeMaxDynamicSharedMemorySize, bytes));
  h->smem_configured.insert(key);
  return MC_OK;
}

template <typename... P, typename... A>
inline void mc_launch(mc_handle* h, void (*kernel)(P...), dim3 grid, dim3 block, size_t smem, cudaStream_t stream, A&&... args) {
  cudaLaunchConfig_t cfg = {};
  cfg.gridDim = grid; cfg.blockDim = block; cfg.dynamicSmemBytes = smem; cfg.stream = stream;
  cudaLaunchAttribute at[1];
  at[0].id = cudaLaunchAttributeProgrammaticStreamSerialization;
  at[0].val.programmaticStreamSerializationAllowed = 1;
  cfg.attrs = at;
  cfg.numAttrs = h->pdl ? 1 : 0;
  (void)cudaLaunchKernelEx(&cfg, kernel, std::forward<A>(args)...);
}

#define MC_LAUNCH_CHECK(h, what)                                                                  \
  do {                                                                                            \
    cudaError_t e__ = cudaGetLastError();                                                         \
    if (e__ != cudaSuccess) return (h)->fail(MC_ERR_CUDA, "launch of %s failed: %s", what, cudaGetErrorString(e__)); \
    (h)->launches++;                                                                              \
  } while (0)

namespace mc_internal {

inline int arena_reserve(mc_handle* h, size_t bytes, cudaStream_t stream) {
  if (bytes <= h->arena_cap) return MC_OK;
  MC_CUDA(h, cudaStreamSynchronize(stream));
  if (h->arena) MC_CUDA(h, cudaFree(h->arena));
  h->arena = nullptr;
  h->arena_cap = 0;
  h->maps.clear();
  const size_t cap = bytes + bytes / 8 + (1u << 20);
  cudaError_t e = cudaMalloc(&h->arena, cap);
  if (e != cudaSuccess) return h->fail(MC_ERR_NOMEM, "workspace cudaMalloc(%zu) failed: %s", cap, cudaGetErrorString(e));
  h->arena_cap = cap;
  return MC_OK;
}
struct Carver {
  size_t off = 0;
  size_t take(size_t bytes) {
    const size_t at = off;
    off += (bytes + 1023) & ~size_t(1023);
    return at;
  }
};

inline int get_map_2d(mc_handle* h, const void* base, int esize, uint64_t dim0, uint64_t dim1, uint64_t row_stride_bytes,
                      uint32_t box0, uint32_t box1, const CUtensorMap** out, int swizzle_bytes = 128) {
  auto key = std::make_tuple(base, dim0, dim1, row_stride_bytes, (uint32_t)(box0 | (esize << 16) | (swizzle_bytes << 20)), box1);
  auto it = h->maps.find(key);
  if (it != h->maps.end()) {
    *out = &it->second;
    return MC_OK;
  }
  EncodeTiledFn enc = get_encode_fn();
  if (!enc) return h->fail(MC_ERR_CUDA, "cuTensorMapEncodeTiled entry point not available");
  if ((reinterpret_cast<uintptr_t>(base) & 15) != 0 || row_stride_bytes % 16 != 0 || box0 * esize > (uint32_t)swizzle_bytes)
    return h->fail(MC_ERR_ARG, "TMA operand misaligned (base %p, row stride %llu B, box %u x %d B)", base,
                   (unsigned long long)row_stride_bytes, box0, esize);
  CUtensorMap m;
  cuuint64_t gdim[2] = {dim0, dim1};
  cuuint64_t gstride[1] = {row_stride_bytes};
  cuuint32_t box[2] = {box0, box1};
  cuuint32_t estride[2] = {1, 1};
  CUresult r = enc(&m, esize == 2 ? CU_TENSOR_MAP_DATA_TYPE_BFLOAT16 : CU_TENSOR_MAP_DATA_TYPE_FLOAT32, 2,
                   const_cast<void*>(base), gdim, gstride, box, estride, CU_TENSOR_MAP_INTERLEAVE_NONE,
                   swizzle_bytes == 32 ? CU_TENSOR_MAP_SWIZZLE_32B : CU_TENSOR_MAP_SWIZZLE_128B, CU_TENSOR_MAP_L2_PROMOTION_L2_256B,
                   CU_TENSOR_MAP_FLOAT_OOB_FILL_NONE);
  if (r != CUDA_SUCCESS)
    return h->fail(MC_ERR_CUDA, "cuTensorMapEncodeTiled failed (%d) dims %llu x %llu box %u x %u esize %d", (int)r,
                   (unsigned long long)dim0, (unsigned long long)dim1, box0, box1, esize);
  auto ins = h->maps.emplace(key, m);
  *out = &ins.first->second;
  return MC_OK;
}
inline int get_map_2d_bf16(mc_handle* h, const void* base, uint64_t dim0, uint64_t dim1, uint32_t box0, uint32_t box1,
                           const CUtensorMap** out, int swizzle_bytes = 128) {
  return get_map_2d(h, base, 2, dim0, dim1, dim0 * 2, box0, box1, out, swizzle_bytes);
}
}
```

### realtime-codec-agent_b200/csrc/gemm_sm100.cuh

```cuda
#pragma once
#include <type_traits>

#include "ptx_sm100.cuh"

namespace mc {

enum : int { ACT_NONE = 0, ACT_GELU_TANH = 1 };
enum : int { OUT_BF16 = 0, OUT_F32 = 1, OUT_F32_RESIDUAL = 2 };

struct GemmParams {
  int M, N, K;
  int a_k_wrap;
  const float* bias;
  int act;
  int out_mode;
  void* out;
  long long ldo;
  int grp_in, grp_valid;
  long long grp_stride, grp_off;
  int tma_store;
  const float* rope_cos;
  int rope_ld;
  const float* rope_sin;
  int rope_cols;
  int rope_period;
  int rope_offset;
  int one = 1;
  const void* prefetch_ptr = nullptr;
  long long prefetch_bytes = 0;
  const float* row_stats = nullptr;
  int row_stats_n = 0;
  float norm_eps = 0.f, inv_norm_dim = 0.f;
  __nv_bfloat16* xb_out = nullptr;
  const float* xb_gamma = nullptr;
  float* stat_out = nullptr;
};

__device__ __forceinline__ float row_rs(const GemmParams& p, int row) {
  const float* st = p.row_stats + static_cast<long long>(row) * p.row_stats_n;
  float s = 0.f;
  for (int c0 = 0; c0 < p.row_stats_n; c0 += 8) {
    float t[8];
#pragma unroll
    for (int j = 0; j < 8; ++j) t[j] = (c0 + j < p.row_stats_n) ? __ldg(st + c0 + j) : 0.f;
#pragma unroll
    for (int j = 0; j < 8; ++j)
      if (c0 + j < p.row_stats_n) s += t[j];
  }
  return rsqrtf(fmaf(s, p.inv_norm_dim, p.norm_eps));
}

constexpr int GEMM_BM = 128;
constexpr int GEMM_BK = 64;
constexpr int GEMM_THREADS = 256;
constexpr int kEpiBufBytes = 4096;

template <int BN>
struct GemmCfg {
  static constexpr int kStageBytesA = GEMM_BM * GEMM_BK * 2;
  static constexpr int kStageBytesB = BN * GEMM_BK * 2;
  static constexpr int kStageBytes = kStageBytesA + kStageBytesB;
  static constexpr int kStages = (BN == 256) ? 4 : (BN == 128 ? 6 : 8);
  static constexpr int kTmemCols = 2 * BN;
  static constexpr int kEpiBytes = 4 * 2 * kEpiBufBytes;
  static constexpr int kBarBytes = 256;
  static constexpr int kSmemBytes = kStages * kStageBytes + kEpiBytes + kBarBytes + 1024;
};

__device__ __forceinline__ float gelu_tanh_f(float x) {
  const float x2 = x * x;
  const float inner = fmaf(x2, 0.7978845608028654f * 0.044715f, 0.7978845608028654f);
  const float u = x * inner;
  float t;
  asm("tanh.approx.f32 %0, %1;" : "=f"(t) : "f"(u));
  const float hx = 0.5f * x;
  return fmaf(hx, t, hx);
}

__device__ __forceinline__ uint32_t pack_bf16x2(float lo, float hi) {
  __nv_bfloat162 h = __floats2bfloat162_rn(lo, hi);
  return *reinterpret_cast<uint32_t*>(&h);
}

struct EpiRegs {
  float bias[64];
  float rc[32], rs[32];
  int rope_pos = -1;
  int buf_sel = 0;
};

template <int BN>
__device__ __forceinline__ void epi_load_bias(const GemmParams& p, int n0, float (&b)[64]) {
#pragma unroll
  for (int j = 0; j < 64; j += 4) {
    float4 b4 = make_float4(0.f, 0.f, 0.f, 0.f);
    if (n0 + j < p.N) b4 = __ldg(reinterpret_cast<const float4*>(p.bias + n0 + j));
    b[j] = b4.x; b[j + 1] = b4.y; b[j + 2] = b4.z; b[j + 3] = b4.w;
  }
}

template <int BN, int RPW = 32>
__device__ __forceinline__ void gemm_epilogue_slab(const GemmParams& p, const CUtensorMap* map_out_p, uint32_t tmem_acc,
                                                   int row_base, int n_base, int q, int lane, uint8_t* my_bufs,
                                                   EpiRegs& st, uint64_t* ready_bar, uint32_t ready_parity) {
  const int g = row_base + q * RPW + (lane < RPW ? lane : 0);
  const int grp = g / p.grp_in;
  const int r = g - grp * p.grp_in;
  const bool row_ok = (lane < RPW) && (g < p.M) && (r < p.grp_valid);
  const long long obase = static_cast<long long>(grp) * p.grp_stride + p.grp_off + static_cast<long long>(r) * p.ldo;
  const bool has_bias = p.bias != nullptr;
  if (has_bias) epi_load_bias<BN>(p, n_base, st.bias);
  const float rs = (p.row_stats != nullptr && g < p.M) ? row_rs(p, g) : 1.0f;
  if (p.rope_period > 0) {
    const int pos = p.rope_offset + r % p.rope_period;
    if (pos != st.rope_pos) {
      st.rope_pos = pos;
#pragma unroll
      for (int j = 0; j < 32; ++j) {
        st.rc[j] = __ldg(p.rope_cos + static_cast<long long>(j) * p.rope_ld + pos);
        st.rs[j] = __ldg(p.rope_sin + static_cast<long long>(j) * p.rope_ld + pos);
      }
    }
  }
  mbar_wait(ready_bar, ready_parity);
  tc_fence_after();

#pragma unroll 1
  for (int c = 0; c < BN / 64; ++c) {
    const int n0 = n_base + c * 64;
    if (n0 >= p.N) break;
    uint32_t raw0[32], raw1[32];
    const uint32_t taddr = tmem_acc + (static_cast<uint32_t>(q * 32) << 16) + c * 64;
    tmem_ld_32x32b_x32(taddr, raw0);
    tmem_ld_32x32b_x32(taddr + 32, raw1);
    tmem_ld_wait();
    float v[64];
#pragma unroll
    for (int j = 0; j < 32; ++j) {
      v[j] = __uint_as_float(raw0[j]);
      v[32 + j] = __uint_as_float(raw1[j]);
    }
    if (p.row_stats != nullptr && has_bias) {
#pragma unroll
      for (int j = 0; j < 64; ++j) v[j] = fmaf(v[j], rs, st.bias[j]);
      if (c + 1 < BN / 64 && n0 + 64 < p.N) epi_load_bias<BN>(p, n0 + 64, st.bias);
    } else if (p.row_stats != nullptr) {
#pragma unroll
      for (int j = 0; j < 64; ++j) v[j] = __fmul_rn(v[j], rs);
    } else if (has_bias) {
#pragma unroll
      for (int j = 0; j < 64; ++j) v[j] += st.bias[j];
      if (c + 1 < BN / 64 && n0 + 64 < p.N) epi_load_bias<BN>(p, n0 + 64, st.bias);
    }
    if (p.act == ACT_GELU_TANH) {
#pragma unroll
      for (int j = 0; j < 64; ++j) v[j] = gelu_tanh_f(v[j]);
    }
    if (p.rope_period > 0 && n0 < p.rope_cols) {
#pragma unroll
      for (int j = 0; j < 32; ++j) {
        const float x1 = v[j], x2 = v[32 + j];
        v[j] = x1 * st.rc[j] - x2 * st.rs[j];
        v[32 + j] = x1 * st.rs[j] + x2 * st.rc[j];
      }
    }
    if (p.tma_store) {
      const int row0 = row_base + q * 32;
      const int sw = lane & 7;
      if (p.out_mode == OUT_BF16) {
        uint8_t* buf = my_bufs + st.buf_sel * kEpiBufBytes;
        if (lane == 0) tma_wait_group_read<1>();
        __syncwarp();
#pragma unroll
        for (int j = 0; j < 8; ++j) {
          uint4 w;
          w.x = pack_bf16x2(v[8 * j], v[8 * j + 1]);
          w.y = pack_bf16x2(v[8 * j + 2], v[8 * j + 3]);
          w.z = pack_bf16x2(v[8 * j + 4], v[8 * j + 5]);
          w.w = pack_bf16x2(v[8 * j + 6], v[8 * j + 7]);
          *reinterpret_cast<uint4*>(buf + lane * 128 + ((j ^ sw) << 4)) = w;
        }
        fence_proxy_async_smem();
        __syncwarp();
        if (lane == 0) {
          tma_store_2d(map_out_p, buf, n0, row0);
          tma_commit_group();
        }
        st.buf_sel ^= 1;
      } else {
#pragma unroll
        for (int half = 0; half < 2; ++half) {
          if (n0 + 32 * half < p.N) {
            uint8_t* buf = my_bufs + st.buf_sel * kEpiBufBytes;
            if (lane == 0) tma_wait_group_read<1>();
            __syncwarp();
#pragma unroll
            for (int j = 0; j < 8; ++j) {
              const float* vv = v + 32 * half + 4 * j;
              *reinterpret_cast<float4*>(buf + lane * 128 + ((j ^ sw) << 4)) = make_float4(vv[0], vv[1], vv[2], vv[3]);
            }
            fence_proxy_async_smem();
            __syncwarp();
            if (lane == 0) {
              if (p.out_mode == OUT_F32_RESIDUAL) tma_reduce_add_2d(map_out_p, buf, n0 + 32 * half, row0);
              else tma_store_2d(map_out_p, buf, n0 + 32 * half, row0);
              tma_commit_group();
            }
            st.buf_sel ^= 1;
          }
        }
      }
    } else if (row_ok) {
      if (p.out_mode == OUT_BF16) {
        __nv_bfloat16* o = reinterpret_cast<__nv_bfloat16*>(p.out) + obase + n0;
#pragma unroll
        for (int j = 0; j < 64; j += 8) {
          if (n0 + j < p.N) {
            uint4 w;
            w.x = pack_bf16x2(v[j], v[j + 1]);
            w.y = pack_bf16x2(v[j + 2], v[j + 3]);
            w.z = pack_bf16x2(v[j + 4], v[j + 5]);
            w.w = pack_bf16x2(v[j + 6], v[j + 7]);
            *reinterpret_cast<uint4*>(o + j) = w;
          }
        }
      } else {
        float* o = reinterpret_cast<float*>(p.out) + obase + n0;
        if (p.xb_out != nullptr) {
          const long long orow = (p.grp_in == INT_MAX) ? g : static_cast<long long>(grp) * p.grp_valid + r;
          __nv_bfloat16* xb = p.xb_out + orow * p.N + n0;
          float gam[64];
#pragma unroll
          for (int j = 0; j < 64; j += 4) {
            float4 ga = make_float4(0.f, 0.f, 0.f, 0.f);
            if (n0 + j < p.N) ga = __ldg(reinterpret_cast<const float4*>(p.xb_gamma + n0 + j));
            gam[j] = ga.x; gam[j + 1] = ga.y; gam[j + 2] = ga.z; gam[j + 3] = ga.w;
          }
          if (p.out_mode == OUT_F32_RESIDUAL) {
#pragma unroll
            for (int j = 0; j < 64; j += 4) {
              if (n0 + j < p.N) {
                const float4 a = *reinterpret_cast<const float4*>(o + j);
                v[j] = __fadd_rn(v[j], a.x); v[j + 1] = __fadd_rn(v[j + 1], a.y); v[j + 2] = __fadd_rn(v[j + 2], a.z); v[j + 3] = __fadd_rn(v[j + 3], a.w);
              }
            }
          }
          float ss = 0.f;
#pragma unroll
          for (int j = 0; j < 64; j += 8) {
            if (n0 + j < p.N) {
              *reinterpret_cast<float4*>(o + j) = make_float4(v[j], v[j + 1], v[j + 2], v[j + 3]);
              *reinterpret_cast<float4*>(o + j + 4) = make_float4(v[j + 4], v[j + 5], v[j + 6], v[j + 7]);
#pragma unroll
              for (int e = 0; e < 8; ++e) ss = fmaf(v[j + e], v[j + e], ss);
              uint4 w;
              w.x = pack_bf16x2(__fmul_rn(v[j], gam[j]), __fmul_rn(v[j + 1], gam[j + 1]));
              w.y = pack_bf16x2(__fmul_rn(v[j + 2], gam[j + 2]), __fmul_rn(v[j + 3], gam[j + 3]));
              w.z = pack_bf16x2(__fmul_rn(v[j + 4], gam[j + 4]), __fmul_rn(v[j + 5], gam[j + 5]));
              w.w = pack_bf16x2(__fmul_rn(v[j + 6], gam[j + 6]), __fmul_rn(v[j + 7], gam[j + 7]));
              *reinterpret_cast<uint4*>(xb + j) = w;
            }
          }
          p.stat_out[orow * ((p.N + 63) / 64) + (n0 >> 6)] = ss;
        } else if (p.out_mode == OUT_F32_RESIDUAL) {
#pragma unroll
          for (int j = 0; j < 64; j += 4) {
            if (n0 + j < p.N) {
              float4 x = *reinterpret_cast<const float4*>(o + j);
              x.x += v[j]; x.y += v[j + 1]; x.z += v[j + 2]; x.w += v[j + 3];
              *reinterpret_cast<float4*>(o + j) = x;
            }
          }
        } else {
#pragma unroll
          for (int j = 0; j < 64; j += 4) {
            if (n0 + j < p.N) {
              *reinterpret_cast<float4*>(o + j) = make_float4(v[j], v[j + 1], v[j + 2], v[j + 3]);
            }
          }
        }
      }
    }
  }
}

enum : int { EPI_GENERIC = 0, EPI_ROPE_BF16 = 1, EPI_GELU_BF16 = 2, EPI_RESID_F32 = 3, EPI_RESID_NORM = 4 };

__device__ __forceinline__ void named_bar_sync(int id, int nthreads) {
  asm volatile("bar.sync %0, %1;" ::"r"(id), "r"(nthreads) : "memory");
}
__device__ __forceinline__ void reg_fence32(uint32_t (&v)[32]) {
  asm volatile(""
               : "+r"(v[0]), "+r"(v[1]), "+r"(v[2]), "+r"(v[3]), "+r"(v[4]), "+r"(v[5]), "+r"(v[6]), "+r"(v[7]),
                 "+r"(v[8]), "+r"(v[9]), "+r"(v[10]), "+r"(v[11]), "+r"(v[12]), "+r"(v[13]), "+r"(v[14]), "+r"(v[15]),
                 "+r"(v[16]), "+r"(v[17]), "+r"(v[18]), "+r"(v[19]), "+r"(v[20]), "+r"(v[21]), "+r"(v[22]), "+r"(v[23]),
                 "+r"(v[24]), "+r"(v[25]), "+r"(v[26]), "+r"(v[27]), "+r"(v[28]), "+r"(v[29]), "+r"(v[30]), "+r"(v[31])
               :
               : "memory");
}

struct EpiFastRegs {
  float rc[32], rs[32];
  int rope_pos = -1;
  int buf_sel = 0;
  float row_scale = 1.0f;
  uint32_t xphase = 0;
};

__device__ __forceinline__ float4 lds_f4(const float* smem_ptr) {
  float4 v;
  asm volatile("ld.shared.v4.f32 {%0, %1, %2, %3}, [%4];" : "=f"(v.x), "=f"(v.y), "=f"(v.z), "=f"(v.w) : "r"(smem_u32(smem_ptr)));
  return v;
}
__device__ __forceinline__ void sts_u4(void* smem_ptr, uint4 w) {
  asm volatile("st.shared.v4.b32 [%0], {%1, %2, %3, %4};" ::"r"(smem_u32(smem_ptr)), "r"(w.x), "r"(w.y), "r"(w.z), "r"(w.w) : "memory");
}

template <int EPI>
__device__ __forceinline__ void epi_fast_chunk(const GemmParams& p, const CUtensorMap* map_out_p, uint32_t (&lo)[32],
                                               uint32_t (&hi)[32], const float* sb ,
                                               int n0, int row0, int lane, uint8_t* my_bufs, EpiFastRegs& st) {
  float v[64];
#pragma unroll
  for (int j = 0; j < 32; ++j) {
    v[j] = __uint_as_float(lo[j]);
    v[32 + j] = __uint_as_float(hi[j]);
  }
  if (p.one != 0) {
#pragma unroll
    if (p.row_stats != nullptr) {
      const float rsc = st.row_scale;
#pragma unroll
      for (int j = 0; j < 32; j += 4) {
        const float4 b0 = lds_f4(sb + j);
        const float4 b1 = lds_f4(sb + 32 + j);
        v[j] = fmaf(v[j], rsc, b0.x); v[j + 1] = fmaf(v[j + 1], rsc, b0.y); v[j + 2] = fmaf(v[j + 2], rsc, b0.z); v[j + 3] = fmaf(v[j + 3], rsc, b0.w);
        v[32 + j] = fmaf(v[32 + j], rsc, b1.x); v[32 + j + 1] = fmaf(v[32 + j + 1], rsc, b1.y);
        v[32 + j + 2] = fmaf(v[32 + j + 2], rsc, b1.z); v[32 + j + 3] = fmaf(v[32 + j + 3], rsc, b1.w);
      }
    } else {
#pragma unroll
      for (int j = 0; j < 32; j += 4) {
        const float4 b0 = lds_f4(sb + j);
        const float4 b1 = lds_f4(sb + 32 + j);
        v[j] += b0.x; v[j + 1] += b0.y; v[j + 2] += b0.z; v[j + 3] += b0.w;
        v[32 + j] += b1.x; v[32 + j + 1] += b1.y; v[32 + j + 2] += b1.z; v[32 + j + 3] += b1.w;
      }
    }
    if (EPI == EPI_GELU_BF16) {
#pragma unroll
      for (int j = 0; j < 64; ++j) v[j] = gelu_tanh_f(v[j]);
    }
    if (EPI == EPI_ROPE_BF16) {
      if (n0 < p.rope_cols) {
#pragma unroll
        for (int j = 0; j < 32; ++j) {
          const float x1 = v[j], x2 = v[32 + j];
          v[j] = x1 * st.rc[j] - x2 * st.rs[j];
          v[32 + j] = x1 * st.rs[j] + x2 * st.rc[j];
        }
      }
    }
  }
  const int sw = lane & 7;
  if (EPI == EPI_RESID_F32) {
#pragma unroll
    for (int half = 0; half < 2; ++half) {
      uint8_t* buf = my_bufs + st.buf_sel * kEpiBufBytes;
      if (lane == 0) tma_wait_group_read<1>();
      __syncwarp();
#pragma unroll
      for (int j = 0; j < 8; ++j) {
        const float* vv = v + 32 * half + 4 * j;
        sts_u4(buf + lane * 128 + ((j ^ sw) << 4), make_uint4(__float_as_uint(vv[0]), __float_as_uint(vv[1]), __float_as_uint(vv[2]),
                                                               __float_as_uint(vv[3])));
      }
      fence_proxy_async_smem();
      __syncwarp();
      if (lane == 0) {
        tma_reduce_add_2d(map_out_p, buf, n0 + 32 * half, row0);
        tma_commit_group();
      }
      st.buf_sel ^= 1;
    }
  } else {
    uint8_t* buf = my_bufs + st.buf_sel * kEpiBufBytes;
    if (lane == 0) tma_wait_group_read<1>();
    __syncwarp();
#pragma unroll
    for (int j = 0; j < 8; ++j) {
      uint4 w;
      w.x = pack_bf16x2(v[8 * j], v[8 * j + 1]);
      w.y = pack_bf16x2(v[8 * j + 2], v[8 * j + 3]);
      w.z = pack_bf16x2(v[8 * j + 4], v[8 * j + 5]);
      w.w = pack_bf16x2(v[8 * j + 6], v[8 * j + 7]);
      sts_u4(buf + lane * 128 + ((j ^ sw) << 4), w);
    }
    fence_proxy_async_smem();
    __syncwarp();
    if (lane == 0) {
      tma_store_2d(map_out_p, buf, n0, row0);
      tma_commit_group();
    }
    st.buf_sel ^= 1;
  }
}

template <int BN, int EPI>
__device__ __forceinline__ void gemm_epilogue_slab_fast(const GemmParams& p, const CUtensorMap* map_out_p, uint32_t tmem_acc,
                                                        int row_base, int n_base, int q, int lane, uint8_t* my_bufs,
                                                        float* sbias , EpiFastRegs& st,
                                                        uint64_t* ready_bar, uint32_t ready_parity) {
  static_assert(BN % 128 == 0, "fast epilogue: chunk pairs");
  named_bar_sync(1, 128);
  {
    const int i = q * 32 + lane;
#pragma unroll
    for (int u = 0; u < BN / 128; ++u) {
      const float bv = __ldg(p.bias + n_base + i * (BN / 128) + u);
      asm volatile("st.shared.f32 [%0], %1;" ::"r"(smem_u32(sbias + i * (BN / 128) + u)), "f"(bv) : "memory");
    }
  }
  if (p.row_stats != nullptr) {
    const int g = row_base + q * 32 + lane;
    st.row_scale = g < p.M ? row_rs(p, g) : 1.0f;
  }
  if (EPI == EPI_ROPE_BF16) {
    if (n_base < p.rope_cols) {
      const int g = row_base + q * 32 + lane;
      const int r = g % p.grp_in;
      const int pos = p.rope_offset + r % p.rope_period;
      if (pos != st.rope_pos) {
        st.rope_pos = pos;
#pragma unroll
        for (int j = 0; j < 32; ++j) {
          st.rc[j] = __ldg(p.rope_cos + static_cast<long long>(j) * p.rope_ld + pos);
          st.rs[j] = __ldg(p.rope_sin + static_cast<long long>(j) * p.rope_ld + pos);
        }
      }
    }
  }
  named_bar_sync(1, 128);
  mbar_wait(ready_bar, ready_parity);
  tc_fence_after();

  const int row0 = row_base + q * 32;
  const uint32_t tbase = tmem_acc + (static_cast<uint32_t>(q * 32) << 16);
  uint32_t a_lo[32], a_hi[32], b_lo[32], b_hi[32];
  tmem_ld_32x32b_x32(tbase, a_lo);
  tmem_ld_32x32b_x32(tbase + 32, a_hi);
  tmem_ld_wait();
  reg_fence32(a_lo);
  reg_fence32(a_hi);
#pragma unroll
  for (int c = 0; c < BN / 64; c += 2) {
    tmem_ld_32x32b_x32(tbase + (c + 1) * 64, b_lo);
    tmem_ld_32x32b_x32(tbase + (c + 1) * 64 + 32, b_hi);
    reg_fence32(a_lo);
    reg_fence32(a_hi);
    epi_fast_chunk<EPI>(p, map_out_p, a_lo, a_hi, sbias + c * 64, n_base + c * 64, row0, lane, my_bufs, st);
    tmem_ld_wait();
    reg_fence32(b_lo);
    reg_fence32(b_hi);
    if (c + 2 < BN / 64) {
      tmem_ld_32x32b_x32(tbase + (c + 2) * 64, a_lo);
      tmem_ld_32x32b_x32(tbase + (c + 2) * 64 + 32, a_hi);
    }
    reg_fence32(b_lo);
    reg_fence32(b_hi);
    epi_fast_chunk<EPI>(p, map_out_p, b_lo, b_hi, sbias + (c + 1) * 64, n_base + (c + 1) * 64, row0, lane, my_bufs, st);
    if (c + 2 < BN / 64) {
      tmem_ld_wait();
      reg_fence32(a_lo);
      reg_fence32(a_hi);
    }
  }
}

template <int BN>
__device__ __forceinline__ void gemm_epilogue_slab_resid_norm(const GemmParams& p, const CUtensorMap* map_x, const CUtensorMap* map_xb,
                                                              uint32_t tmem_acc, int row_base, int n_base, int q, int lane,
                                                              uint8_t* wbuf , uint64_t* xbar ,
                                                              float* sbias , EpiFastRegs& st,
                                                              uint64_t* ready_bar, uint32_t ready_parity) {
  static_assert(BN % 128 == 0, "chunk pairs");
  named_bar_sync(1, 128);
  {
    const int i = q * 32 + lane;
#pragma unroll
    for (int u = 0; u < BN / 128; ++u) {
      const int n = i * (BN / 128) + u;
      asm volatile("st.shared.f32 [%0], %1;" ::"r"(smem_u32(sbias + n)), "f"(__ldg(p.bias + n_base + n)) : "memory");
      asm volatile("st.shared.f32 [%0], %1;" ::"r"(smem_u32(sbias + BN + n)), "f"(__ldg(p.xb_gamma + n_base + n)) : "memory");
    }
  }
  const int row0 = row_base + q * 32;
  const int g = row0 + lane;
  uint8_t* xb0 = wbuf;
  uint8_t* bf0 = wbuf + 4 * kEpiBufBytes;
  if (lane == 0) {
    tma_wait_group_read<0>();
#pragma unroll
    for (int set = 0; set < 2; ++set) {
      mbar_arrive_expect_tx(&xbar[set], 2 * kEpiBufBytes);
      tma_load_2d(xb0 + (set * 2) * kEpiBufBytes, map_x, &xbar[set], n_base + set * 64, row0);
      tma_load_2d(xb0 + (set * 2 + 1) * kEpiBufBytes, map_x, &xbar[set], n_base + set * 64 + 32, row0);
    }
  }
  named_bar_sync(1, 128);
  mbar_wait(ready_bar, ready_parity);
  tc_fence_after();
  const uint32_t tbase = tmem_acc + (static_cast<uint32_t>(q * 32) << 16);
  const int sw = lane & 7;
  const int nst = p.N >> 6;
#pragma unroll 1
  for (int c = 0; c < BN / 64; ++c) {
    const int set = c & 1;
    const int n0 = n_base + c * 64;
    uint32_t lo[32], hi[32];
    tmem_ld_32x32b_x32(tbase + c * 64, lo);
    tmem_ld_32x32b_x32(tbase + c * 64 + 32, hi);
    tmem_ld_wait();
    mbar_wait(&xbar[set], (st.xphase >> set) & 1u);
    st.xphase ^= (1u << set);
    float v[64];
    const float* sb = sbias + c * 64;
#pragma unroll
    for (int hf = 0; hf < 2; ++hf) {
      uint8_t* xbox = xb0 + (set * 2 + hf) * kEpiBufBytes + lane * 128;
#pragma unroll
      for (int j = 0; j < 8; ++j) {
        const float4 xo = lds_f4(reinterpret_cast<const float*>(xbox + ((j ^ sw) << 4)));
        const float4 bb = lds_f4(sb + hf * 32 + 4 * j);
        const uint32_t* a = (hf == 0 ? lo : hi) + 4 * j;
        float* vv = v + hf * 32 + 4 * j;
        vv[0] = __fadd_rn(__fadd_rn(__uint_as_float(a[0]), bb.x), xo.x);
        vv[1] = __fadd_rn(__fadd_rn(__uint_as_float(a[1]), bb.y), xo.y);
        vv[2] = __fadd_rn(__fadd_rn(__uint_as_float(a[2]), bb.z), xo.z);
        vv[3] = __fadd_rn(__fadd_rn(__uint_as_float(a[3]), bb.w), xo.w);
      }
    }
    float ss = 0.f;
#pragma unroll
    for (int j = 0; j < 64; ++j) ss = fmaf(v[j], v[j], ss);
    if (g < p.M) p.stat_out[static_cast<long long>(g) * nst + (n0 >> 6)] = ss;
#pragma unroll
    for (int hf = 0; hf < 2; ++hf) {
      uint8_t* xbox = xb0 + (set * 2 + hf) * kEpiBufBytes + lane * 128;
#pragma unroll
      for (int j = 0; j < 8; ++j) {
        const float* vv = v + hf * 32 + 4 * j;
        sts_u4(xbox + ((j ^ sw) << 4), make_uint4(__float_as_uint(vv[0]), __float_as_uint(vv[1]), __float_as_uint(vv[2]), __float_as_uint(vv[3])));
      }
    }
    if (lane == 0) tma_wait_group_read<0>();
    __syncwarp();
    {
      uint8_t* bbox = bf0 + lane * 128;
      const float* sg = sbias + BN + c * 64;
#pragma unroll
      for (int j = 0; j < 8; ++j) {
        const float4 g0 = lds_f4(sg + 8 * j), g1 = lds_f4(sg + 8 * j + 4);
        uint4 w;
        w.x = pack_bf16x2(__fmul_rn(v[8 * j], g0.x), __fmul_rn(v[8 * j + 1], g0.y));
        w.y = pack_bf16x2(__fmul_rn(v[8 * j + 2], g0.z), __fmul_rn(v[8 * j + 3], g0.w));
        w.z = pack_bf16x2(__fmul_rn(v[8 * j + 4], g1.x), __fmul_rn(v[8 * j + 5], g1.y));
        w.w = pack_bf16x2(__fmul_rn(v[8 * j + 6], g1.z), __fmul_rn(v[8 * j + 7], g1.w));
        sts_u4(bbox + ((j ^ sw) << 4), w);
      }
    }
    fence_proxy_async_smem();
    __syncwarp();
    if (lane == 0) {
      tma_store_2d(map_x, xb0 + (set * 2) * kEpiBufBytes, n0, row0);
      tma_store_2d(map_x, xb0 + (set * 2 + 1) * kEpiBufBytes, n0 + 32, row0);
      tma_store_2d(map_xb, bf0, n0, row0);
      tma_commit_group();
      if (c + 2 < BN / 64) {
        tma_wait_group_read<0>();
        mbar_arrive_expect_tx(&xbar[set], 2 * kEpiBufBytes);
        tma_load_2d(xb0 + (set * 2) * kEpiBufBytes, map_x, &xbar[set], n0 + 128, row0);
        tma_load_2d(xb0 + (set * 2 + 1) * kEpiBufBytes, map_x, &xbar[set], n0 + 128 + 32, row0);
      }
    }
    __syncwarp();
  }
}

template <int BN, int BM = GEMM_BM, int KPS = 1>
__global__ void __launch_bounds__(GEMM_THREADS, 1)
gemm_bf16_sm100_kernel(const __grid_constant__ CUtensorMap map_a, const __grid_constant__ CUtensorMap map_b,
                       const __grid_constant__ CUtensorMap map_out, const GemmParams p) {
  using Cfg = GemmCfg<BN>;
  constexpr int kStagesK = Cfg::kStages / KPS;
  constexpr int kStageBytesK = Cfg::kStageBytes * KPS;
  static_assert(Cfg::kStages % KPS == 0 && kStagesK >= 2, "stage grouping");
  extern __shared__ uint8_t smem_raw[];
  uint8_t* smem = reinterpret_cast<uint8_t*>((reinterpret_cast<uintptr_t>(smem_raw) + 1023) & ~uintptr_t(1023));
  uint8_t* epi_base = smem + Cfg::kStages * Cfg::kStageBytes;
  uint8_t* bar_base = epi_base + Cfg::kEpiBytes;
  uint64_t* full_bar = reinterpret_cast<uint64_t*>(bar_base);
  uint64_t* empty_bar = full_bar + Cfg::kStages;
  uint64_t* tmem_full = empty_bar + Cfg::kStages;
  uint64_t* tmem_empty = tmem_full + 2;
  uint32_t* tmem_ptr = reinterpret_cast<uint32_t*>(tmem_empty + 2);

  const int warp = threadIdx.x >> 5;
  const int lane = threadIdx.x & 31;
  const int m_tiles = (p.M + BM - 1) / BM;
  const int n_tiles = (p.N + BN - 1) / BN;
  const int num_tiles = m_tiles * n_tiles;
  const int num_kb = p.K / GEMM_BK;
  constexpr uint32_t kTxBytes = (BM * GEMM_BK * 2 + Cfg::kStageBytesB) * KPS;

  if (warp == 4 && lane == 0) {
    tma_prefetch_desc(&map_a);
    tma_prefetch_desc(&map_b);
    if (p.tma_store) tma_prefetch_desc(&map_out);
  }
  if (warp == 5 && lane == 0) {
    for (int s = 0; s < kStagesK; ++s) {
      mbar_init(&full_bar[s], 1);
      mbar_init(&empty_bar[s], 1);
    }
    for (int s = 0; s < 2; ++s) {
      mbar_init(&tmem_full[s], 1);
      mbar_init(&tmem_empty[s], 4);
    }
    fence_mbar_init();
  }
  if (warp == 6) {
    tmem_alloc(tmem_ptr, Cfg::kTmemCols);
    tmem_relinquish();
  }
  pdl_launch_dependents();
  tc_fence_before();
  __syncthreads();
  tc_fence_after();
  const uint32_t tmem_base = *tmem_ptr;
  pdl_wait();

  if (warp == 4) {
    if (lane == 0) {
      int stage = 0;
      uint32_t phase = 0;
      for (int tile = blockIdx.x; tile < num_tiles; tile += gridDim.x) {
        const int m_blk = tile / n_tiles, n_blk = tile % n_tiles;
        for (int kb = 0; kb < num_kb; kb += KPS) {
          mbar_wait(&empty_bar[stage], phase ^ 1);
          mbar_arrive_expect_tx(&full_bar[stage], kTxBytes);
#pragma unroll
          for (int j = 0; j < KPS; ++j) {
            uint8_t* sa = smem + stage * kStageBytesK + j * Cfg::kStageBytes;
            uint8_t* sb = sa + Cfg::kStageBytesA;
            const int k_elem = (kb + j) * GEMM_BK;
            const int row_off = k_elem / p.a_k_wrap;
            const int a_k = k_elem - row_off * p.a_k_wrap;
            tma_load_2d(sa, &map_a, &full_bar[stage], a_k, m_blk * BM + row_off);
            tma_load_2d(sb, &map_b, &full_bar[stage], k_elem, n_blk * BN);
          }
          if (++stage == kStagesK) { stage = 0; phase ^= 1; }
        }
      }
    }
  } else if (warp == 5) {
    if (lane == 0) {
      constexpr uint32_t idesc = umma_idesc_bf16(BM, BN, 0, 0);
      int stage = 0;
      uint32_t phase = 0;
      int it = 0;
      for (int tile = blockIdx.x; tile < num_tiles; tile += gridDim.x, ++it) {
        const int acc = it & 1;
        const uint32_t acc_phase = (it >> 1) & 1;
        mbar_wait(&tmem_empty[acc], acc_phase ^ 1);
        tc_fence_after();
        const uint32_t d_tmem = tmem_base + acc * BN;
        for (int kb = 0; kb < num_kb; kb += KPS) {
          mbar_wait(&full_bar[stage], phase);
          tc_fence_after();
#pragma unroll
          for (int j = 0; j < KPS; ++j) {
            const uint32_t sa = smem_u32(smem + stage * kStageBytesK + j * Cfg::kStageBytes);
            const uint32_t sb = sa + Cfg::kStageBytesA;
            const uint64_t adesc = umma_smem_desc_sw128(sa, 1024, 16);
            const uint64_t bdesc = umma_smem_desc_sw128(sb, 1024, 16);
#pragma unroll
            for (int k = 0; k < GEMM_BK / 16; ++k) {
              umma_bf16_ss(d_tmem, adesc + 2 * k, bdesc + 2 * k, idesc, (kb | j | k) != 0);
            }
          }
          umma_commit(&empty_bar[stage]);
          if (++stage == kStagesK) { stage = 0; phase ^= 1; }
        }
        umma_commit(&tmem_full[acc]);
      }
    }
  } else if (warp < 4) {
    const int q = warp;
    uint8_t* my_bufs = epi_base + q * 2 * kEpiBufBytes;
    EpiRegs st;
    int it = 0;
    for (int tile = blockIdx.x; tile < num_tiles; tile += gridDim.x, ++it) {
      const int m_blk = tile / n_tiles, n_blk = tile % n_tiles;
      const int acc = it & 1;
      const uint32_t acc_phase = (it >> 1) & 1;
      gemm_epilogue_slab<BN, BM / 4>(p, &map_out, tmem_base + acc * BN, m_blk * BM, n_blk * BN, q, lane, my_bufs, st,
                                     &tmem_full[acc], acc_phase);
      tc_fence_before();
      __syncwarp();
      if (lane == 0) mbar_arrive(&tmem_empty[acc]);
    }
    if (p.tma_store && lane == 0) tma_wait_group_read<0>();
  }

  __syncwarp();
  tc_fence_before();
  __syncthreads();
  if (warp == 6) {
    tc_fence_after();
    tmem_dealloc(tmem_base, Cfg::kTmemCols);
  }
}


template <int BN, int EPI = EPI_GENERIC>
struct Gemm2Cfg {
  static constexpr int kStageBytesA = GEMM_BM * GEMM_BK * 2;
  static constexpr int kStageBytesB = (BN / 2) * GEMM_BK * 2;
  static constexpr int kStageBytes = kStageBytesA + kStageBytesB;
  static constexpr int kEpiBytes = (EPI == EPI_RESID_NORM ? 4 * 5 : 4 * 2) * kEpiBufBytes;
  static constexpr int kStages = (EPI == EPI_RESID_NORM ? 131072 : 196608) / kStageBytes;
  static constexpr int kTmemCols = 2 * BN;
  static constexpr int kBarBytes = 256;
  static constexpr int kBiasBytes = (EPI == EPI_RESID_NORM ? 2 : 1) * BN * 4;
  static constexpr int kSmemBytes = kStages * kStageBytes + kEpiBytes + kBarBytes + kBiasBytes + 1024;
  static_assert(kSmemBytes <= 232448, "CTA-pair GEMM exceeds 227 KB of shared memory");
};

template <int BN, int EPI>
__global__ void __cluster_dims__(2, 1, 1) __launch_bounds__(GEMM_THREADS, 1)
gemm2_bf16_sm100_kernel(const __grid_constant__ CUtensorMap map_a, const __grid_constant__ CUtensorMap map_b,
                        const __grid_constant__ CUtensorMap map_out, const __grid_constant__ CUtensorMap map_out2, const GemmParams p) {
  using Cfg = Gemm2Cfg<BN, EPI>;
  extern __shared__ uint8_t smem_raw[];
  uint8_t* smem = reinterpret_cast<uint8_t*>((reinterpret_cast<uintptr_t>(smem_raw) + 1023) & ~uintptr_t(1023));
  uint8_t* epi_base = smem + Cfg::kStages * Cfg::kStageBytes;
  uint8_t* bar_base = epi_base + Cfg::kEpiBytes;
  uint64_t* full_bar = reinterpret_cast<uint64_t*>(bar_base);
  uint64_t* empty_bar = full_bar + Cfg::kStages;
  uint64_t* tmem_full = empty_bar + Cfg::kStages;
  uint64_t* tmem_empty = tmem_full + 2;
  uint64_t* xbar = tmem_empty + 2;
  uint32_t* tmem_ptr = reinterpret_cast<uint32_t*>(xbar + 8);
  float* sbias = reinterpret_cast<float*>(bar_base + Cfg::kBarBytes);

  const int warp = threadIdx.x >> 5;
  const int lane = threadIdx.x & 31;
  const uint32_t rank = cluster_ctarank();
  const int pair = blockIdx.x >> 1, num_pairs = gridDim.x >> 1;
  const int m_tiles = (p.M + 2 * GEMM_BM - 1) / (2 * GEMM_BM);
  const int n_tiles = (p.N + BN - 1) / BN;
  const int num_tiles = m_tiles * n_tiles;
  const int num_kb = p.K / GEMM_BK;

  if (warp == 4 && lane == 0) {
    tma_prefetch_desc(&map_a);
    tma_prefetch_desc(&map_b);
    if (p.tma_store) tma_prefetch_desc(&map_out);
    if (EPI == EPI_RESID_NORM) tma_prefetch_desc(&map_out2);
  }
  if (warp == 5 && lane == 0) {
    for (int s = 0; s < Cfg::kStages; ++s) {
      mbar_init(&full_bar[s], 2);
      mbar_init(&empty_bar[s], 1);
    }
    for (int s = 0; s < 2; ++s) {
      mbar_init(&tmem_full[s], 1);
      mbar_init(&tmem_empty[s], 8);
    }
    for (int s = 0; s < 8; ++s) mbar_init(&xbar[s], 1);
    fence_mbar_init();
  }
  if (warp == 6) {
    tmem_alloc_pair(tmem_ptr, Cfg::kTmemCols);
    tmem_relinquish_pair();
  }
  pdl_launch_dependents();
  tc_fence_before();
  __syncthreads();
  cluster_sync_all();
  tc_fence_after();
  const uint32_t tmem_base = *tmem_ptr;
  pdl_wait();

  if (warp == 4) {
    if (lane == 0) {
      int stage = 0;
      uint32_t phase = 0;
      for (int tile = pair; tile < num_tiles; tile += num_pairs) {
        const int m_blk = tile / n_tiles, n_blk = tile % n_tiles;
        for (int kb = 0; kb < num_kb; ++kb) {
          mbar_wait(&empty_bar[stage], phase ^ 1);
          uint8_t* sa = smem + stage * Cfg::kStageBytes;
          uint8_t* sb = sa + Cfg::kStageBytesA;
          const uint32_t leader_full = mapa_shared(smem_u32(&full_bar[stage]), 0);
          if (rank == 0) mbar_arrive_expect_tx(&full_bar[stage], 2 * Cfg::kStageBytes);
          else mbar_arrive_cluster(leader_full);
          const int k_elem = kb * GEMM_BK;
          const int row_off = k_elem / p.a_k_wrap;
          const int a_k = k_elem - row_off * p.a_k_wrap;
          tma_load_2d_pair(sa, &map_a, leader_full, a_k, m_blk * 2 * GEMM_BM + rank * GEMM_BM + row_off);
          tma_load_2d_pair(sb, &map_b, leader_full, k_elem, n_blk * BN + rank * (BN / 2));
          if (++stage == Cfg::kStages) { stage = 0; phase ^= 1; }
        }
      }
    }
  } else if (warp == 5) {
    if (lane == 0 && rank == 0) {
      constexpr uint32_t idesc = umma_idesc_bf16(2 * GEMM_BM, BN, 0, 0);
      int stage = 0;
      uint32_t phase = 0;
      int it = 0;
      for (int tile = pair; tile < num_tiles; tile += num_pairs, ++it) {
        const int acc = it & 1;
        const uint32_t acc_phase = (it >> 1) & 1;
        mbar_wait(&tmem_empty[acc], acc_phase ^ 1);
        tc_fence_after();
        const uint32_t d_tmem = tmem_base + acc * BN;
        for (int kb = 0; kb < num_kb; ++kb) {
          mbar_wait(&full_bar[stage], phase);
          tc_fence_after();
          const uint32_t sa = smem_u32(smem + stage * Cfg::kStageBytes);
          const uint32_t sb = sa + Cfg::kStageBytesA;
          const uint64_t adesc = umma_smem_desc_sw128(sa, 1024, 16);
          const uint64_t bdesc = umma_smem_desc_sw128(sb, 1024, 16);
#pragma unroll
          for (int k = 0; k < GEMM_BK / 16; ++k) umma_bf16_ss_pair(d_tmem, adesc + 2 * k, bdesc + 2 * k, idesc, (kb | k) != 0);
          umma_commit_pair(&empty_bar[stage], 3);
          if (++stage == Cfg::kStages) { stage = 0; phase ^= 1; }
        }
        umma_commit_pair(&tmem_full[acc], 3);
      }
    }
  } else if (warp < 4) {
    const int q = warp;
    uint8_t* my_bufs = epi_base + q * (EPI == EPI_RESID_NORM ? 5 : 2) * kEpiBufBytes;
    typename std::conditional<EPI == EPI_GENERIC, EpiRegs, EpiFastRegs>::type st;
    int it = 0;
    for (int tile = pair; tile < num_tiles; tile += num_pairs, ++it) {
      const int m_blk = tile / n_tiles, n_blk = tile % n_tiles;
      const int acc = it & 1;
      const uint32_t acc_phase = (it >> 1) & 1;
      if constexpr (EPI == EPI_GENERIC) {
        gemm_epilogue_slab<BN>(p, &map_out, tmem_base + acc * BN, m_blk * 2 * GEMM_BM + rank * GEMM_BM, n_blk * BN, q, lane,
                               my_bufs, st, &tmem_full[acc], acc_phase);
      } else if constexpr (EPI == EPI_RESID_NORM) {
        gemm_epilogue_slab_resid_norm<BN>(p, &map_out, &map_out2, tmem_base + acc * BN, m_blk * 2 * GEMM_BM + rank * GEMM_BM,
                                          n_blk * BN, q, lane, my_bufs, xbar + 2 * q, sbias, st, &tmem_full[acc], acc_phase);
      } else {
        gemm_epilogue_slab_fast<BN, EPI>(p, &map_out, tmem_base + acc * BN, m_blk * 2 * GEMM_BM + rank * GEMM_BM, n_blk * BN, q,
                                         lane, my_bufs, sbias, st, &tmem_full[acc], acc_phase);
      }
      tc_fence_before();
      __syncwarp();
      if (lane == 0) mbar_arrive_cluster(mapa_shared(smem_u32(&tmem_empty[acc]), 0));
    }
    if (p.tma_store && lane == 0) tma_wait_group_read<0>();
  }

  __syncwarp();
  tc_fence_before();
  __syncthreads();
  cluster_sync_all();
  if (warp == 6) {
    tc_fence_after();
    tmem_dealloc_pair(tmem_base, Cfg::kTmemCols);
  }
}

}
```

Measured before the change: 5635.

## Compute layer-0 QKV once on shared stem and fan out to overlapping windows

With a shared stem, the first encoder layer's norm and QKV projection are computed once over the unique span frames. A new GEMM epilogue then fans each row out, applying per-window RoPE positions, to every overlapping window's qkv buffer through TMA stores. Pre-pad rows get a separate small norm and GEMM. This removes the redundant layer-0 QKV GEMM over duplicated overlapping rows, at the cost of a more complex epilogue with multiple stores per row, fewer pipeline stages and extra shared memory for a RoPE table.

Result: faster. 5743, median of 6 (+1.9%).

```diff
diff --git a/realtime-codec-agent_b200/csrc/elementwise.cuh b/realtime-codec-agent_b200/csrc/elementwise.cuh
--- a/realtime-codec-agent_b200/csrc/elementwise.cuh
+++ b/realtime-codec-agent_b200/csrc/elementwise.cuh
@@ -50,15 +50,18 @@
   }
 }
 
+template <bool kRemapX>
 __global__ void rmsnorm_kernel(const float* __restrict__ x, const float* __restrict__ gamma,
                                __nv_bfloat16* __restrict__ out, int M, int d, float eps, int grp_in,
-                               long long grp_stride, long long grp_off) {
+                               long long grp_stride, long long grp_off, int x_grp, long long x_grp_stride) {
   pdl_launch_dependents();
   pdl_wait();
   const int warps_per_block = blockDim.x >> 5;
   const int lane = threadIdx.x & 31;
   for (int row = blockIdx.x * warps_per_block + (threadIdx.x >> 5); row < M; row += gridDim.x * warps_per_block) {
-    const float4* xr = reinterpret_cast<const float4*>(x + static_cast<long long>(row) * d);
+    const float* xrow = x + static_cast<long long>(row) * d;
+    if (kRemapX) xrow = x + (row / x_grp) * x_grp_stride + static_cast<long long>(row % x_grp) * d;
+    const float4* xr = reinterpret_cast<const float4*>(xrow);
     const int n4 = d >> 2;
     float ss = 0.0f;
     for (int i = lane; i < n4; i += 32) {
@@ -83,10 +86,10 @@
   }
 }
 
-template <int NV>
+template <int NV, bool kRemapX>
 __global__ void __launch_bounds__(256)
 rmsnorm_rows_kernel(const float* __restrict__ x, const float* __restrict__ gamma, __nv_bfloat16* __restrict__ out, int M,
-                    float eps, int grp_in, long long grp_stride, long long grp_off) {
+                    float eps, int grp_in, long long grp_stride, long long grp_off, int x_grp, long long x_grp_stride) {
   pdl_launch_dependents();
   pdl_wait();
   constexpr int d = NV * 128;
@@ -96,7 +99,9 @@
 #pragma unroll
   for (int u = 0; u < NV; ++u) g[u] = __ldg(reinterpret_cast<const float4*>(gamma) + lane + 32 * u);
   for (int row = blockIdx.x * warps_per_block + (threadIdx.x >> 5); row < M; row += gridDim.x * warps_per_block) {
-    const float4* xr = reinterpret_cast<const float4*>(x + static_cast<long long>(row) * d);
+    const float* xrow = x + static_cast<long long>(row) * d;
+    if (kRemapX) xrow = x + (row / x_grp) * x_grp_stride + static_cast<long long>(row % x_grp) * d;
+    const float4* xr = reinterpret_cast<const float4*>(xrow);
     float4 v[NV];
 #pragma unroll
     for (int u = 0; u < NV; ++u) v[u] = xr[lane + 32 * u];
diff --git a/realtime-codec-agent_b200/csrc/engine.cu b/realtime-codec-agent_b200/csrc/engine.cu
--- a/realtime-codec-agent_b200/csrc/engine.cu
+++ b/realtime-codec-agent_b200/csrc/engine.cu
@@ -116,6 +116,36 @@
   if (fast_ok && c.out_mode == OUT_F32_RESIDUAL && c.act == ACT_NONE && c.rope_period == 0 && c.xb_out == nullptr)
     return launch_gemm_pair_epi<EPI_RESID_F32>(h, p, ma, mb, mo, mo2, pairs, stream);
   return launch_gemm_pair_epi<EPI_GENERIC>(h, p, ma, mb, mo, mo2, pairs, stream);
+}
+
+bool pair_selected(const mc_handle* h, long long M, int N) {
+  return h->gemm_pair && N >= 256 && ((M + 255) / 256) * ((N + 255) / 256) >= h->num_sms / 2;
+}
+
+int launch_qkv_fanout(mc_handle* h, const bf16* A, int S, const bf16* W, const float* bias, bf16* qkv, int B, int F, int pre,
+                      int step, cudaStream_t stream) {
+  constexpr int BN = 256;
+  const int d = h->spec.d_model, N = 3 * d;
+  if (N % BN != 0 || F > kFanMaxPos || F > h->spec.max_positions || pre >= F || step < 1)
+    return h->fail(MC_ERR_ARG, "qkv fan-out: unsupported shape (3d %d, F %d, pre %d, step %d)", N, F, pre, step);
+  const CUtensorMap *ma, *mb, *mo;
+  MC_TRY(get_map_2d_bf16(h, A, (uint64_t)d, (uint64_t)S, GEMM_BK, GEMM_BM, &ma));
+  MC_TRY(get_map_2d_bf16(h, W, (uint64_t)d, (uint64_t)N, GEMM_BK, BN / 2, &mb));
+  MC_TRY(get_map_2d(h, qkv, 2, (uint64_t)N, (uint64_t)B * F, (uint64_t)N * 2, 64, 32, &mo));
+  GemmParams p;
+  p.tma_store = 1;
+  p.M = S; p.N = N; p.K = d; p.a_k_wrap = d;
+  p.bias = bias; p.act = ACT_NONE; p.out_mode = OUT_BF16; p.out = qkv; p.ldo = N;
+  p.grp_in = INT_MAX; p.grp_valid = INT_MAX; p.grp_stride = 0; p.grp_off = 0;
+  p.rope_cols = 2 * d; p.rope_period = F; p.rope_offset = 0;
+  p.rope_ld = h->spec.max_positions;
+  p.rope_cos = h->ptr<float>("rope.cos");
+  p.rope_sin = h->ptr<float>("rope.sin");
+  p.fan_step = step; p.fan_F = F; p.fan_pre = pre; p.fan_B = B;
+  const int m_tiles = (S + 2 * GEMM_BM - 1) / (2 * GEMM_BM), n_tiles = N / BN;
+  const int pairs = std::min(m_tiles * n_tiles, h->num_sms / 2);
+  McProfScope prof(h, 0, 2.0 * S * N * d, (double)S * d * 2.0 + (double)N * d * 2.0 + (double)B * (F - pre) * N * 2.0, stream);
+  return launch_gemm_pair_epi<EPI_ROPE_FANOUT>(h, p, ma, mb, mo, mo, pairs, stream);
 }
 
 template <int S>
@@ -198,10 +228,7 @@
     const int S = pick_split_k(h, c);
     if (S >= 2) return launch_gemm_splitk(h, c, S, stream);
   }
-  {
-    const int m2 = (c.M + 255) / 256, n2 = (c.N + 255) / 256;
-    if ((bn == 0 && h->gemm_pair && c.N >= 256 && m2 * n2 >= h->num_sms / 2) || bn == 512) return launch_gemm_pair(h, c, stream);
-  }
+  if ((bn == 0 && pair_selected(h, c.M, c.N)) || bn == 512) return launch_gemm_pair(h, c, stream);
   if (bn == 0) {
     const int m_tiles = (c.M + GEMM_BM - 1) / GEMM_BM;
     if (c.N >= 256 && m_tiles * ((c.N + 255) / 256) >= 2 * h->num_sms) bn = 256;
@@ -228,20 +255,29 @@
   return (int)blocks;
 }
 
-int launch_rmsnorm(mc_handle* h, const float* x, const float* gamma, bf16* out, int M, int d, int grp_in,
-                   int64_t grp_stride, int64_t grp_off, cudaStream_t stream) {
-  if (d % 4 != 0) return h->fail(MC_ERR_ARG, "rmsnorm: d=%d must be a multiple of 4", d);
+template <bool kRemapX>
+void launch_rmsnorm_kernel(mc_handle* h, const float* x, const float* gamma, bf16* out, int M, int d, int grp_in, long long grp_stride,
+                           long long grp_off, int x_grp, long long x_grp_stride, cudaStream_t stream) {
   const int warps = 8;
   const int grid = ew_grid(h, M, warps);
-  McProfScope prof(h, 3, 0.0, (double)M * d * 6.0, stream);
   const float eps = h->spec.norm_eps;
   switch (d % 128 == 0 ? d / 128 : 0) {
-    case 1: mc_launch(h, rmsnorm_rows_kernel<1>, dim3(grid), dim3(warps * 32), 0, stream, x, gamma, out, M, eps, grp_in, (long long)grp_stride, (long long)grp_off); break;
-    case 2: mc_launch(h, rmsnorm_rows_kernel<2>, dim3(grid), dim3(warps * 32), 0, stream, x, gamma, out, M, eps, grp_in, (long long)grp_stride, (long long)grp_off); break;
-    case 4: mc_launch(h, rmsnorm_rows_kernel<4>, dim3(grid), dim3(warps * 32), 0, stream, x, gamma, out, M, eps, grp_in, (long long)grp_stride, (long long)grp_off); break;
-    case 8: mc_launch(h, rmsnorm_rows_kernel<8>, dim3(grid), dim3(warps * 32), 0, stream, x, gamma, out, M, eps, grp_in, (long long)grp_stride, (long long)grp_off); break;
-    default: mc_launch(h, rmsnorm_kernel, dim3(grid), dim3(warps * 32), 0, stream, x, gamma, out, M, d, eps, grp_in, (long long)grp_stride, (long long)grp_off);
-  }
+    case 1: mc_launch(h, rmsnorm_rows_kernel<1, kRemapX>, dim3(grid), dim3(warps * 32), 0, stream, x, gamma, out, M, eps, grp_in, grp_stride, grp_off, x_grp, x_grp_stride); break;
+    case 2: mc_launch(h, rmsnorm_rows_kernel<2, kRemapX>, dim3(grid), dim3(warps * 32), 0, stream, x, gamma, out, M, eps, grp_in, grp_stride, grp_off, x_grp, x_grp_stride); break;
+    case 4: mc_launch(h, rmsnorm_rows_kernel<4, kRemapX>, dim3(grid), dim3(warps * 32), 0, stream, x, gamma, out, M, eps, grp_in, grp_stride, grp_off, x_grp, x_grp_stride); break;
+    case 8: mc_launch(h, rmsnorm_rows_kernel<8, kRemapX>, dim3(grid), dim3(warps * 32), 0, stream, x, gamma, out, M, eps, grp_in, grp_stride, grp_off, x_grp, x_grp_stride); break;
+    default: mc_launch(h, rmsnorm_kernel<kRemapX>, dim3(grid), dim3(warps * 32), 0, stream, x, gamma, out, M, d, eps, grp_in, grp_stride, grp_off, x_grp, x_grp_stride);
+  }
+}
+
+int launch_rmsnorm(mc_handle* h, const float* x, const float* gamma, bf16* out, int M, int d, int grp_in,
+                   int64_t grp_stride, int64_t grp_off, cudaStream_t stream, int x_grp = INT_MAX, int64_t x_grp_stride = 0) {
+  if (d % 4 != 0) return h->fail(MC_ERR_ARG, "rmsnorm: d=%d must be a multiple of 4", d);
+  McProfScope prof(h, 3, 0.0, (double)M * d * 6.0, stream);
+  if (x_grp == INT_MAX)
+    launch_rmsnorm_kernel<false>(h, x, gamma, out, M, d, grp_in, (long long)grp_stride, (long long)grp_off, x_grp, (long long)x_grp_stride, stream);
+  else
+    launch_rmsnorm_kernel<true>(h, x, gamma, out, M, d, grp_in, (long long)grp_stride, (long long)grp_off, x_grp, (long long)x_grp_stride, stream);
   MC_LAUNCH_CHECK(h, "rmsnorm_kernel");
   return MC_OK;
 }
@@ -294,7 +330,7 @@
 
 int run_layers(mc_handle* h, const char* prefix, int n_layers, const StackBufs& b, int B, int F, int keep_rows,
                float** x_out, cudaStream_t stream, int fuse_mode = 0 ,
-               const float* final_gamma = nullptr, bf16** xb_out = nullptr, float** stats_out = nullptr) {
+               const float* final_gamma = nullptr, bf16** xb_out = nullptr, float** stats_out = nullptr, bool qkv0_ready = false) {
   const mc_spec& s = h->spec;
   const int d = s.d_model, f = s.ffn_dim;
   const int nst = d / 64;
@@ -322,14 +358,16 @@
     };
     const int Ri = rows, Ro = std::min(r_out[l], rows);
     const int Mi = B * Ri, Mo = B * Ro;
-    if (!fused) MC_TRY(launch_rmsnorm(h, x, h->ptr<float>(T("norm1")), b.hbuf, Mi, d, INT_MAX, 0, 0, stream));
-    GemmCall g{};
-    if (fused) { g.row_stats = b.stats; g.row_stats_n = nst; }
-    g.A = b.hbuf; g.a_rows = Mi; g.a_k_wrap = d; g.W = h->ptr<bf16>(T("wqkv")); g.bias = h->ptr<float>(T("bqkv"));
-    g.M = Mi; g.N = 3 * d; g.K = d; g.act = ACT_NONE; g.out_mode = OUT_BF16; g.out = b.qkv; g.ldo = 3 * d;
-    g.rope_cols = 2 * d; g.rope_period = Ri; g.rope_offset = F - Ri;
-    g.prefetch_ptr = h->ptr<bf16>(T("wo")); g.prefetch_bytes = (long long)d * d * 2;
-    MC_TRY(launch_gemm(h, g, stream));
+    if (l > 0 || !qkv0_ready) {
+      if (!fused) MC_TRY(launch_rmsnorm(h, x, h->ptr<float>(T("norm1")), b.hbuf, Mi, d, INT_MAX, 0, 0, stream));
+      GemmCall g{};
+      if (fused) { g.row_stats = b.stats; g.row_stats_n = nst; }
+      g.A = b.hbuf; g.a_rows = Mi; g.a_k_wrap = d; g.W = h->ptr<bf16>(T("wqkv")); g.bias = h->ptr<float>(T("bqkv"));
+      g.M = Mi; g.N = 3 * d; g.K = d; g.act = ACT_NONE; g.out_mode = OUT_BF16; g.out = b.qkv; g.ldo = 3 * d;
+      g.rope_cols = 2 * d; g.rope_period = Ri; g.rope_offset = F - Ri;
+      g.prefetch_ptr = h->ptr<bf16>(T("wo")); g.prefetch_bytes = (long long)d * d * 2;
+      MC_TRY(launch_gemm(h, g, stream));
+    }
     MC_TRY(launch_attention(h, b.qkv, b.att, B, Ri, Ro, (F - Ri) % 16, h->attn_impl, stream));
     if (Ro < Ri) {
       const long long items = (long long)Mo * (d / 4);
@@ -536,14 +574,18 @@
   const int fuse_mode = !(fuse_norm_ok(h, Mll + B) && s.enc_layers > 0) ? 0 : ((h->fuse_norm == 3 && !few_rows_regime(h, Mll + B)) ? 2 : 1);
   const bool fused = fuse_mode == 1;
   const bool conv_producer = fused && few_rows_regime(h, Mll + B) && !shared;
+  const bool shared_qkv = shared && h->shared_qkv && fuse_mode == 0 && s.enc_layers > 0 && h->fast_epilogue &&
+                          !(h->split_k == 2 || (h->split_k == 1 && h->in_session)) && (3 * d) % 256 == 0 &&
+                          F <= kFanMaxPos && pair_selected(h, span_frames, 3 * d);
 
   Carver cv;
   ConvPlan cp_full, cp_span, cp_pre;
-  size_t ostem = 0;
+  size_t ostem = 0, onorm = 0;
   if (shared) {
     cp_span = plan_conv(s, cv, 1, (int)span_samples);
     cp_pre = plan_conv(s, cv, B, pre * hop);
     ostem = cv.take((size_t)span_frames * d * 4);
+    if (shared_qkv) onorm = cv.take((size_t)(span_frames + (long long)pre * B) * d * 2);
   } else {
     cp_full = plan_conv(s, cv, B, Tp);
   }
@@ -567,6 +609,22 @@
     mc_launch(h, gather_stem_kernel, dim3(ew_grid(h, items, 256)), dim3(256), 0, stream, reinterpret_cast<const float4*>(stem),
               reinterpret_cast<float4*>(sb.x), B, F, pre, (int)(ld / hop), d / 4);
     MC_LAUNCH_CHECK(h, "gather_stem_kernel");
+    if (shared_qkv) {
+      const float* g1 = h->ptr<float>("enc.layers.0.norm1");
+      const bf16* wqkv = h->ptr<bf16>("enc.layers.0.wqkv");
+      const float* bqkv = h->ptr<float>("enc.layers.0.bqkv");
+      bf16* xn = reinterpret_cast<bf16*>(base + onorm);
+      bf16* xn_pre = xn + (size_t)span_frames * d;
+      MC_TRY(launch_rmsnorm(h, stem, g1, xn, (int)span_frames, d, INT_MAX, 0, 0, stream));
+      MC_TRY(launch_rmsnorm(h, sb.x, g1, xn_pre, pre * B, d, INT_MAX, 0, 0, stream, pre, (int64_t)F * d));
+      MC_TRY(launch_qkv_fanout(h, xn, (int)span_frames, wqkv, bqkv, sb.qkv, B, F, pre, (int)(ld / hop), stream));
+      GemmCall g{};
+      g.A = xn_pre; g.a_rows = pre * B; g.a_k_wrap = d; g.W = wqkv; g.bias = bqkv;
+      g.M = pre * B; g.N = 3 * d; g.K = d; g.act = ACT_NONE; g.out_mode = OUT_BF16; g.out = sb.qkv; g.ldo = 3 * d;
+      g.grp_in = pre; g.grp_valid = pre; g.grp_stride = (int64_t)F * 3 * d; g.grp_off = 0;
+      g.rope_cols = 2 * d; g.rope_period = pre; g.rope_offset = 0;
+      MC_TRY(launch_gemm(h, g, stream));
+    }
   } else {
     if (conv_producer)
       MC_TRY(run_conv_stack(h, cp_full, base, wav, ld, T, sb.x, (int64_t)F * d, stream, sb.hbuf, h->ptr<float>("enc.layers.0.norm1"), sb.stats));
@@ -578,7 +636,8 @@
   float* xk = nullptr;
   bf16* xbk = sb.hbuf;
   float* stk = nullptr;
-  MC_TRY(run_layers(h, "enc", s.enc_layers, sb, B, F, keep_rows, &xk, stream, fuse_mode, fused ? h->ptr<float>("enc.norm_f") : nullptr, &xbk, &stk));
+  MC_TRY(run_layers(h, "enc", s.enc_layers, sb, B, F, keep_rows, &xk, stream, fuse_mode, fused ? h->ptr<float>("enc.norm_f") : nullptr, &xbk,
+                    &stk, shared_qkv));
   const int Mk = B * keep_rows;
   if (!fused) MC_TRY(launch_rmsnorm(h, xk, h->ptr<float>("enc.norm_f"), sb.hbuf, Mk, d, INT_MAX, 0, 0, stream));
   GemmCall pj{};
@@ -983,6 +1042,7 @@
   const std::string k(key);
   if (k == "shared_stem") h->shared_stem = value != 0;
   else if (k == "exact_cut") { h->exact_cut = value != 0; h->tensor_gen++; }
+  else if (k == "shared_qkv") h->shared_qkv = value != 0;
   else if (k == "gemm_pair") h->gemm_pair = value != 0;
   else if (k == "fast_epilogue") h->fast_epilogue = value != 0;
   else if (k == "pdl") h->pdl = value != 0;
diff --git a/realtime-codec-agent_b200/csrc/engine_common.cuh b/realtime-codec-agent_b200/csrc/engine_common.cuh
--- a/realtime-codec-agent_b200/csrc/engine_common.cuh
+++ b/realtime-codec-agent_b200/csrc/engine_common.cuh
@@ -70,6 +70,7 @@
   bool pdl = true;
   bool shared_stem = true;
   bool exact_cut = true;
+  bool shared_qkv = true;
   struct ProfRec { cudaEvent_t a, b; int cls; double flops; double bytes; };
   bool profiling = false;
   std::vector<ProfRec> prof;
diff --git a/realtime-codec-agent_b200/csrc/gemm_sm100.cuh b/realtime-codec-agent_b200/csrc/gemm_sm100.cuh
--- a/realtime-codec-agent_b200/csrc/gemm_sm100.cuh
+++ b/realtime-codec-agent_b200/csrc/gemm_sm100.cuh
@@ -34,6 +34,7 @@
   __nv_bfloat16* xb_out = nullptr;
   const float* xb_gamma = nullptr;
   float* stat_out = nullptr;
+  int fan_step = 0, fan_F = 0, fan_pre = 0, fan_B = 0;
 };
 
 __device__ __forceinline__ float row_rs(const GemmParams& p, int row) {
@@ -80,6 +81,11 @@
 __device__ __forceinline__ uint32_t pack_bf16x2(float lo, float hi) {
   __nv_bfloat162 h = __floats2bfloat162_rn(lo, hi);
   return *reinterpret_cast<uint32_t*>(&h);
+}
+
+__device__ __forceinline__ void rope_rotate(float x1, float x2, float c, float s, float& y1, float& y2) {
+  y1 = __fmaf_rn(x1, c, -__fmul_rn(x2, s));
+  y2 = __fmaf_rn(x1, s, __fmul_rn(x2, c));
 }
 
 struct EpiRegs {
@@ -284,7 +290,9 @@
   }
 }
 
-enum : int { EPI_GENERIC = 0, EPI_ROPE_BF16 = 1, EPI_GELU_BF16 = 2, EPI_RESID_F32 = 3, EPI_RESID_NORM = 4 };
+enum : int { EPI_GENERIC = 0, EPI_ROPE_BF16 = 1, EPI_GELU_BF16 = 2, EPI_RESID_F32 = 3, EPI_RESID_NORM = 4, EPI_ROPE_FANOUT = 5 };
+constexpr int kFanBufs = 4;
+constexpr int kFanMaxPos = 128;
 
 __device__ __forceinline__ void named_bar_sync(int id, int nthreads) {
   asm volatile("bar.sync %0, %1;" ::"r"(id), "r"(nthreads) : "memory");
@@ -473,6 +481,156 @@
       tmem_ld_wait();
       reg_fence32(a_lo);
       reg_fence32(a_hi);
+    }
+  }
+}
+
+__device__ __forceinline__ void fan_stage_rope(const GemmParams& p, float* tab, int tid ) {
+  for (int i = tid; i < p.fan_F * 64; i += 128) {
+    const int t = i % p.fan_F, e = i / p.fan_F;
+    const float v = __ldg((e < 32 ? p.rope_cos : p.rope_sin) + static_cast<long long>(e & 31) * p.rope_ld + t);
+    tab[t * 64 + (((e >> 2) ^ (t & 7)) << 2) + (e & 3)] = v;
+  }
+}
+
+static_assert(kFanBufs == 4, "fan_acquire_box waits on at most three later groups");
+struct FanRegs {
+  int buf_sel = 0;
+  uint32_t hist = 0;
+};
+
+__device__ __forceinline__ void fan_acquire_box(const FanRegs& st, int lane) {
+  if (lane == 0 && ((st.hist >> (kFanBufs - 1)) & 1u)) {
+    switch (__popc(st.hist & ((1u << (kFanBufs - 1)) - 1u))) {
+      case 0: tma_wait_group_read<0>(); break;
+      case 1: tma_wait_group_read<1>(); break;
+      case 2: tma_wait_group_read<2>(); break;
+      default: tma_wait_group_read<3>(); break;
+    }
+  }
+  __syncwarp();
+}
+
+__device__ __forceinline__ void fan_release_box(FanRegs& st, bool stored_by_tma, int lane) {
+  if (stored_by_tma && lane == 0) tma_commit_group();
+  st.hist = ((st.hist << 1) | (stored_by_tma ? 1u : 0u)) & ((1u << kFanBufs) - 1u);
+  st.buf_sel = st.buf_sel + 1 == kFanBufs ? 0 : st.buf_sel + 1;
+}
+
+__device__ __forceinline__ bool fan_store_box(const GemmParams& p, const CUtensorMap* map_out_p, const uint8_t* buf, int n0,
+                                              int w, int r0, int lane) {
+  const int rows = p.fan_F - p.fan_pre;
+  if (r0 >= 0 && r0 + 32 <= rows) {
+    if (lane == 0) tma_store_2d(map_out_p, buf, n0, w * p.fan_F + p.fan_pre + r0);
+    return true;
+  }
+  const int ch = lane & 7;
+  __nv_bfloat16* out = reinterpret_cast<__nv_bfloat16*>(p.out) + (static_cast<long long>(w) * p.fan_F + p.fan_pre) * p.ldo + n0 + ch * 8;
+#pragma unroll
+  for (int k = 0; k < 8; ++k) {
+    const int i = 4 * k + (lane >> 3);
+    const int t = r0 + i;
+    if (t >= 0 && t < rows) {
+      uint4 u;
+      asm volatile("ld.shared.v4.b32 {%0, %1, %2, %3}, [%4];"
+                   : "=r"(u.x), "=r"(u.y), "=r"(u.z), "=r"(u.w)
+                   : "r"(smem_u32(buf + i * 128 + ((ch ^ (i & 7)) << 4))));
+      *reinterpret_cast<uint4*>(out + static_cast<long long>(t) * p.ldo) = u;
+    }
+  }
+  return false;
+}
+
+template <int BN>
+__device__ __forceinline__ void gemm_epilogue_slab_fanout(const GemmParams& p, const CUtensorMap* map_out_p, uint32_t tmem_acc,
+                                                          int row_base, int n_base, int q, int lane, uint8_t* my_bufs,
+                                                          float* sbias, const float* rtab, FanRegs& st,
+                                                          uint64_t* ready_bar, uint32_t ready_parity) {
+  named_bar_sync(1, 128);
+  {
+    const int i = q * 32 + lane;
+#pragma unroll
+    for (int u = 0; u < BN / 128; ++u) {
+      const float bv = __ldg(p.bias + n_base + i * (BN / 128) + u);
+      asm volatile("st.shared.f32 [%0], %1;" ::"r"(smem_u32(sbias + i * (BN / 128) + u)), "f"(bv) : "memory");
+    }
+  }
+  named_bar_sync(1, 128);
+  const int row0 = row_base + q * 32;
+  const int step = p.fan_step, F = p.fan_F, pre = p.fan_pre;
+  const int lo_num = row0 - (F - 1);
+  const int w_lo = lo_num <= 0 ? 0 : (lo_num + step - 1) / step;
+  const int w_hi = min(p.fan_B - 1, (row0 + 31 - pre) / step);
+  mbar_wait(ready_bar, ready_parity);
+  tc_fence_after();
+  const uint32_t tbase = tmem_acc + (static_cast<uint32_t>(q * 32) << 16);
+  const int f = row0 + lane;
+  const int sw = lane & 7;
+#pragma unroll 1
+  for (int c = 0; c < BN / 64; ++c) {
+    const int n0 = n_base + c * 64;
+    uint32_t lo[32], hi[32];
+    tmem_ld_32x32b_x32(tbase + c * 64, lo);
+    tmem_ld_32x32b_x32(tbase + c * 64 + 32, hi);
+    tmem_ld_wait();
+    float v[64];
+#pragma unroll
+    for (int j = 0; j < 32; ++j) {
+      v[j] = __uint_as_float(lo[j]);
+      v[32 + j] = __uint_as_float(hi[j]);
+    }
+    const float* sb = sbias + c * 64;
+#pragma unroll
+    for (int j = 0; j < 32; j += 4) {
+      const float4 b0 = lds_f4(sb + j);
+      const float4 b1 = lds_f4(sb + 32 + j);
+      v[j] += b0.x; v[j + 1] += b0.y; v[j + 2] += b0.z; v[j + 3] += b0.w;
+      v[32 + j] += b1.x; v[32 + j + 1] += b1.y; v[32 + j + 2] += b1.z; v[32 + j + 3] += b1.w;
+    }
+    if (n0 < p.rope_cols) {
+#pragma unroll 1
+      for (int w = w_lo; w <= w_hi; ++w) {
+        const int tc = min(max(f - step * w, 0), F - 1);
+        const float* tr = rtab + tc * 64;
+        const int tsw = tc & 7;
+        uint8_t* buf = my_bufs + st.buf_sel * kEpiBufBytes;
+        fan_acquire_box(st, lane);
+#pragma unroll
+        for (int jb = 0; jb < 4; ++jb) {
+          const float4 c0 = lds_f4(tr + (((2 * jb) ^ tsw) << 2)), c1 = lds_f4(tr + (((2 * jb + 1) ^ tsw) << 2));
+          const float4 s0 = lds_f4(tr + (((8 + 2 * jb) ^ tsw) << 2)), s1 = lds_f4(tr + (((9 + 2 * jb) ^ tsw) << 2));
+          const float cs[8] = {c0.x, c0.y, c0.z, c0.w, c1.x, c1.y, c1.z, c1.w};
+          const float sn[8] = {s0.x, s0.y, s0.z, s0.w, s1.x, s1.y, s1.z, s1.w};
+          float y1[8], y2[8];
+#pragma unroll
+          for (int e = 0; e < 8; ++e) rope_rotate(v[8 * jb + e], v[32 + 8 * jb + e], cs[e], sn[e], y1[e], y2[e]);
+          sts_u4(buf + lane * 128 + ((jb ^ sw) << 4),
+                 make_uint4(pack_bf16x2(y1[0], y1[1]), pack_bf16x2(y1[2], y1[3]), pack_bf16x2(y1[4], y1[5]), pack_bf16x2(y1[6], y1[7])));
+          sts_u4(buf + lane * 128 + (((jb + 4) ^ sw) << 4),
+                 make_uint4(pack_bf16x2(y2[0], y2[1]), pack_bf16x2(y2[2], y2[3]), pack_bf16x2(y2[4], y2[5]), pack_bf16x2(y2[6], y2[7])));
+        }
+        fence_proxy_async_smem();
+        __syncwarp();
+        fan_release_box(st, fan_store_box(p, map_out_p, buf, n0, w, row0 - step * w - pre, lane), lane);
+      }
+    } else {
+      uint8_t* buf = my_bufs + st.buf_sel * kEpiBufBytes;
+      fan_acquire_box(st, lane);
+#pragma unroll
+      for (int j = 0; j < 8; ++j) {
+        uint4 wv;
+        wv.x = pack_bf16x2(v[8 * j], v[8 * j + 1]);
+        wv.y = pack_bf16x2(v[8 * j + 2], v[8 * j + 3]);
+        wv.z = pack_bf16x2(v[8 * j + 4], v[8 * j + 5]);
+        wv.w = pack_bf16x2(v[8 * j + 6], v[8 * j + 7]);
+        sts_u4(buf + lane * 128 + ((j ^ sw) << 4), wv);
+      }
+      fence_proxy_async_smem();
+      __syncwarp();
+      bool any_tma = false;
+#pragma unroll 1
+      for (int w = w_lo; w <= w_hi; ++w) any_tma |= fan_store_box(p, map_out_p, buf, n0, w, row0 - step * w - pre, lane);
+      fan_release_box(st, any_tma, lane);
     }
   }
 }
@@ -728,12 +886,14 @@
   static constexpr int kStageBytesA = GEMM_BM * GEMM_BK * 2;
   static constexpr int kStageBytesB = (BN / 2) * GEMM_BK * 2;
   static constexpr int kStageBytes = kStageBytesA + kStageBytesB;
-  static constexpr int kEpiBytes = (EPI == EPI_RESID_NORM ? 4 * 5 : 4 * 2) * kEpiBufBytes;
-  static constexpr int kStages = (EPI == EPI_RESID_NORM ? 131072 : 196608) / kStageBytes;
+  static constexpr int kEpiBufs = EPI == EPI_RESID_NORM ? 5 : (EPI == EPI_ROPE_FANOUT ? kFanBufs : 2);
+  static constexpr int kEpiBytes = 4 * kEpiBufs * kEpiBufBytes;
+  static constexpr int kStages = (EPI == EPI_RESID_NORM || EPI == EPI_ROPE_FANOUT ? 131072 : 196608) / kStageBytes;
   static constexpr int kTmemCols = 2 * BN;
   static constexpr int kBarBytes = 256;
   static constexpr int kBiasBytes = (EPI == EPI_RESID_NORM ? 2 : 1) * BN * 4;
-  static constexpr int kSmemBytes = kStages * kStageBytes + kEpiBytes + kBarBytes + kBiasBytes + 1024;
+  static constexpr int kRopeBytes = EPI == EPI_ROPE_FANOUT ? kFanMaxPos * 64 * 4 : 0;
+  static constexpr int kSmemBytes = kStages * kStageBytes + kEpiBytes + kBarBytes + kBiasBytes + kRopeBytes + 1024;
   static_assert(kSmemBytes <= 232448, "CTA-pair GEMM exceeds 227 KB of shared memory");
 };
 
@@ -753,6 +913,7 @@
   uint64_t* xbar = tmem_empty + 2;
   uint32_t* tmem_ptr = reinterpret_cast<uint32_t*>(xbar + 8);
   float* sbias = reinterpret_cast<float*>(bar_base + Cfg::kBarBytes);
+  float* rtab = sbias + Cfg::kBiasBytes / 4;
 
   const int warp = threadIdx.x >> 5;
   const int lane = threadIdx.x & 31;
@@ -844,8 +1005,10 @@
     }
   } else if (warp < 4) {
     const int q = warp;
-    uint8_t* my_bufs = epi_base + q * (EPI == EPI_RESID_NORM ? 5 : 2) * kEpiBufBytes;
-    typename std::conditional<EPI == EPI_GENERIC, EpiRegs, EpiFastRegs>::type st;
+    uint8_t* my_bufs = epi_base + q * Cfg::kEpiBufs * kEpiBufBytes;
+    typename std::conditional<EPI == EPI_GENERIC, EpiRegs,
+                              typename std::conditional<EPI == EPI_ROPE_FANOUT, FanRegs, EpiFastRegs>::type>::type st;
+    if constexpr (EPI == EPI_ROPE_FANOUT) fan_stage_rope(p, rtab, q * 32 + lane);
     int it = 0;
     for (int tile = pair; tile < num_tiles; tile += num_pairs, ++it) {
       const int m_blk = tile / n_tiles, n_blk = tile % n_tiles;
@@ -854,6 +1017,9 @@
       if constexpr (EPI == EPI_GENERIC) {
         gemm_epilogue_slab<BN>(p, &map_out, tmem_base + acc * BN, m_blk * 2 * GEMM_BM + rank * GEMM_BM, n_blk * BN, q, lane,
                                my_bufs, st, &tmem_full[acc], acc_phase);
+      } else if constexpr (EPI == EPI_ROPE_FANOUT) {
+        gemm_epilogue_slab_fanout<BN>(p, &map_out, tmem_base + acc * BN, m_blk * 2 * GEMM_BM + rank * GEMM_BM, n_blk * BN, q,
+                                      lane, my_bufs, sbias, rtab, st, &tmem_full[acc], acc_phase);
       } else if constexpr (EPI == EPI_RESID_NORM) {
         gemm_epilogue_slab_resid_norm<BN>(p, &map_out, &map_out2, tmem_base + acc * BN, m_blk * 2 * GEMM_BM + rank * GEMM_BM,
                                           n_blk * BN, q, lane, my_bufs, xbar + 2 * q, sbias, st, &tmem_full[acc], acc_phase);
```
